# haileys/mixlab

Hardware: AMD Instinct MI355X
Metric: audio_ch_mixed_per_sec (higher is better)
Workload: dtype f32 (f64 intermediates); 1 GPU; 1024-channel Mixer + EqThree + Envelope chain (Trigger->Envelope; noise->EqThree->StereoPanner->Amplifier->Mixer), 48000 Hz f32; strips=1024, gates=toggle every 30 ticks, phase k mod 60, applied between ticks inside the batch, eq_mode=exact order: speculative time-parallel kernel, verified bit-exact, parallelism=strips sharded x1, ticks_policy=one GPU

## Files before the change

include/mixlab_gpu.h:

```cpp
#ifndef MIXLAB_GPU_H
#define MIXLAB_GPU_H

#include <stddef.h>
#include <stdint.h>

#ifdef __cplusplus
extern "C" {
#endif

#define MX_ABI_VERSION 4u

enum {
    MX_OK = 0,
    MX_ERR_INVALID = -1,
    MX_ERR_TYPE = -2,
    MX_ERR_DEVICE = -3,
    MX_ERR_NOMEM = -4,
    MX_ERR_INTERNAL = -5,
    MX_ERR_FULL = -6
};

typedef enum { MX_DISCONNECTED = 0, MX_MONO = 1, MX_STEREO = 2, MX_VIDEO = 3 } mx_line;

enum {
// ... 11 lines not shown
    MX_KIND_SOURCE_MONO = 11,
    MX_KIND_SOURCE_STEREO = 12,
    MX_KIND_SOURCE_VIDEO = 13,
    MX_KIND_VIDEO_TO_RGBA = 14,
    MX_KIND_FIR = 15,
    MX_KIND_RESAMPLE = 16,
    MX_KIND_MONITOR = 17,
    MX_KIND_OUTPUT_DEVICE = 18,
    MX_KIND_COUNT = 19
};
#define MX_PROFILE_KINDS 18

enum { MX_WAVE_ON = 0, MX_WAVE_OFF = 1, MX_WAVE_SINE = 2, MX_WAVE_SQUARE = 3, MX_WAVE_TRIANGLE = 4, MX_WAVE_SAW = 5 };

typedef struct { double gain_db; double fader; uint8_t cue; uint8_t _pad[7]; } mx_mixer_channel_params;
typedef struct { double gain_lo_db, gain_mid_db, gain_hi_db; } mx_eq_three_params;
typedef struct { double attack_ms, decay_ms, sustain_amplitude, release_ms; } mx_envelope_params;
typedef struct { double amplitude, mod_depth; } mx_amplifier_params;
typedef struct { double freq; uint32_t waveform; uint32_t _pad; } mx_oscillator_params;
typedef struct { double freq_lo, freq_hi; } mx_fm_sine_params;
typedef struct { uint32_t gate_open; } mx_trigger_params;
typedef struct { int32_t a, b;  double fader; } mx_video_mixer_params;
typedef struct { int32_t use_matrix; int32_t matrix_q12[12]; } mx_video_to_rgba_params;
typedef struct { uint32_t width, height; } mx_monitor_params;
typedef struct { uint32_t width, height, queue_depth, _pad; } mx_monitor_params_ex;
typedef struct { uint32_t channels; int32_t left, right; uint32_t _pad; } mx_output_device_params;
typedef struct { uint32_t n_taps; uint32_t _pad;  } mx_fir_params;
typedef struct { uint32_t up, down, taps_per_phase, _pad;  } mx_resample_params;

typedef struct { uint32_t kind; uint32_t params_len; const void* params; } mx_node;
typedef struct { uint32_t src_node, src_port, dst_node, dst_port; } mx_edge;

#define MX_FLAG_EQ_EXACT 1u
#define MX_FLAG_EQ_FAST 4u
#define MX_FLAG_FP_CONTRACT 16u

#define MX_FLAG_OVERLAP_TAIL 8u
#define MX_FLAG_NO_FUSE 2u

typedef struct {
    uint32_t sample_rate;
    uint32_t ticks_per_second;
    uint32_t max_ticks_per_run;
    uint32_t flags;
    int32_t device;
    int32_t _pad;
    void* stream;
} mx_graph_opts;

typedef struct mx_graph mx_graph;

const char* mx_last_error(void);
uint32_t mx_abi_version(void);
int mx_device_count(void);

int mx_graph_build(const mx_node* nodes, size_t n_nodes, const mx_edge* edges, size_t n_edges,
                   const mx_graph_opts* opts, mx_graph** out);
void mx_graph_destroy(mx_graph* g);

int mx_graph_samples_per_tick(const mx_graph* g, size_t* spt);
int mx_graph_run_order(const mx_graph* g, uint32_t* order, size_t cap, size_t* n);

int mx_graph_stream(mx_graph* g, void** stream);
int mx_graph_tail_stream(mx_graph* g, void** stream);

int mx_graph_update_params(mx_graph* g, uint32_t node, const void* params, size_t params_len);

typedef struct { uint32_t node; uint32_t tick_in_run; const void* params; size_t params_len; } mx_param_event;
int mx_graph_schedule_params(mx_graph* g, uint32_t node, uint32_t tick_in_run, const void* params, size_t params_len);
int mx_graph_schedule_params_batch(mx_graph* g, const mx_param_event* events, size_t n_events);

int mx_graph_eq_spec_stats(mx_graph* g, uint64_t* chunks_run, uint64_t* chunks_repaired);
int mx_graph_eq_repair_stats(mx_graph* g, uint64_t out[8]);
int mx_graph_debug_eq_records(mx_graph* g, void** device_records, size_t* bytes);
int mx_graph_debug_tail_releases(mx_graph* g, uint64_t* gated, uint64_t* at_once);
#define MX_EQ_LAUNCH_NONE 0u
#define MX_EQ_LAUNCH_SEQUENTIAL 1u
#define MX_EQ_LAUNCH_DIRECT 2u
#define MX_EQ_LAUNCH_TILED 3u
#define MX_EQ_LAUNCH_RAGGED_TICK 4u
#define MX_EQ_LAUNCH_CONTROL_TILE 5u
#define MX_EQ_LAUNCH_SCAN 6u
int mx_graph_debug_eq_launch(mx_graph* g, uint32_t out[5]);

int mx_graph_write_source(mx_graph* g, uint32_t node, const float* host_samples, size_t n_ticks);
int mx_graph_bind_source_device(mx_graph* g, uint32_t node, const void* device_ptr);

int mx_graph_run_ticks(mx_graph* g, uint64_t first_tick, uint32_t n_ticks);
int mx_graph_sync(mx_graph* g);

int mx_graph_read_output(mx_graph* g, uint32_t node, uint32_t port, float* host_samples, size_t n_ticks);
int mx_graph_read_output_window(mx_graph* g, uint32_t node, uint32_t port, float* host_samples, size_t first_tick_in_run, size_t n_ticks);
int mx_graph_read_output_i16(mx_graph* g, uint32_t node, uint32_t port, int16_t* host_samples, size_t n_ticks);
int mx_graph_write_source_i16(mx_graph* g, uint32_t node, const int16_t* host_samples, size_t n_ticks);

int mx_graph_output_device_ptr(mx_graph* g, uint32_t node, uint32_t port, void** device_ptr, size_t* floats_per_tick);

typedef struct { uint8_t clip, clip_status, lag_status, changed; uint32_t channels; } mx_audio_out_tick;
int mx_graph_read_audio_out(mx_graph* g, uint32_t node, uint32_t first_tick_in_run, uint32_t n_ticks, float* samples, size_t samples_cap,
                            mx_audio_out_tick* ticks, size_t* n_samples);
int mx_graph_audio_out_lag(mx_graph* g, uint32_t node);

typedef struct { uint32_t node, port; } mx_port_ref;
typedef struct { uint32_t hold_ticks; float release; } mx_meter_params;
typedef struct {
    float    peak[2];
    float    hold[2];
    double   sum_sq[2];
    uint32_t over[2];
    uint32_t frames;
    uint32_t channels;
} mx_meter_tick;
int mx_graph_set_meters(mx_graph* g, const mx_port_ref* ports, size_t n, const mx_meter_params* params);
int mx_graph_read_meters(mx_graph* g, uint32_t first_tick_in_run, uint32_t n_ticks, mx_meter_tick* dst, size_t cap);

typedef struct {
    uint32_t        n_fft;
    uint32_t        n_bands;
    const uint16_t* edges;
} mx_spectrum_params;
int mx_graph_set_spectra(mx_graph* g, const mx_port_ref* ports, size_t n, const mx_spectrum_params* params);
int mx_graph_read_spectra(mx_graph* g, uint32_t first_tick_in_run, uint32_t n_ticks, float* dst, size_t cap);
int mx_spectrum_tables(uint32_t n_fft, float* window, float* twiddle_re, float* twiddle_im);

typedef struct { uint32_t momentary_ticks; uint32_t short_ticks; } mx_loudness_params;
typedef struct {
    double   ksq[2];
    double   momentary_sq;
    double   short_sq;
    float    true_peak[2];
    uint32_t frames;
    uint32_t channels;
} mx_loudness_tick;
int mx_graph_set_loudness(mx_graph* g, const mx_port_ref* ports, size_t n, const mx_loudness_params* params);
int mx_graph_read_loudness(mx_graph* g, uint32_t first_tick_in_run, uint32_t n_ticks, mx_loudness_tick* dst, size_t cap);
int mx_loudness_tables(double rate, uint32_t frames_per_tick, double* biquads, double* carry, float* interp);
int mx_loudness_gate(const double* block_sq, const uint32_t* block_frames, size_t n_blocks, double* lufs_integrated, size_t* blocks_kept);

typedef struct { uint32_t window_ticks , grid , zoom_log2 , hop ; } mx_stereo_params;
typedef struct {
    double   sum_ll;
    double   sum_rr;
    double   sum_lr;
    double   win_ll;
    double   win_rr;
    double   win_lr;
    uint32_t frames;
    uint32_t nonfinite;
} mx_stereo_tick;
int mx_graph_set_stereo(mx_graph* g, const mx_port_ref* ports, size_t n, const mx_stereo_params* params);
int mx_graph_read_stereo(mx_graph* g, uint32_t first_tick_in_run, uint32_t n_ticks, mx_stereo_tick* dst, size_t cap);
int mx_graph_read_goniometers(mx_graph* g, void* dst, size_t cap_bytes, uint32_t* n_records);
int mx_stereo_gonio_record_bytes(const mx_stereo_params* params, size_t* bytes);
int mx_stereo_correlation(double ll, double rr, double lr, double* r);

typedef struct { float ceiling; uint32_t lookahead; } mx_limiter_params;
#define MX_LIMITER_MAX_LOOKAHEAD 512u
typedef struct {
    float    min_gain;
    float    peak_out;
    uint32_t limited;
    uint32_t nonfinite;
    uint32_t frames;
    uint32_t channels;
} mx_limiter_tick;
int mx_graph_set_limiters(mx_graph* g, const mx_port_ref* ports, size_t n, const mx_limiter_params* params);
// ... 227 lines not shown
```

mixlab_amd/abi.py:

```python
from __future__ import annotations

import ctypes as C
import pathlib

import numpy as np

_PKG = pathlib.Path(__file__).resolve().parent
LIB_PATH = _PKG / "libmixlab_gpu.so"

if not LIB_PATH.exists():
    raise ImportError(
        f"{LIB_PATH} is missing: build it with `python -m mixlab_amd.build` (hipcc, gfx950). "
        "mixlab_amd has no CPU fallback."
    )

lib = C.CDLL(str(LIB_PATH))

MX_OK, MX_ERR_INVALID, MX_ERR_TYPE, MX_ERR_DEVICE, MX_ERR_NOMEM, MX_ERR_INTERNAL, MX_ERR_FULL = 0, -1, -2, -3, -4, -5, -6
MX_DISCONNECTED, MX_MONO, MX_STEREO, MX_VIDEO = 0, 1, 2, 3
(KIND_AMPLIFIER, KIND_ENVELOPE, KIND_EQ_THREE, KIND_FM_SINE, KIND_MIXER, KIND_OSCILLATOR, KIND_PLOTTER,
 KIND_STEREO_PANNER, KIND_STEREO_SPLITTER, KIND_TRIGGER, KIND_VIDEO_MIXER, KIND_SOURCE_MONO,
 KIND_SOURCE_STEREO, KIND_SOURCE_VIDEO, KIND_VIDEO_TO_RGBA, KIND_FIR, KIND_RESAMPLE, KIND_MONITOR, KIND_OUTPUT_DEVICE, KIND_COUNT) = range(20)
PROFILE_KINDS = 18
KIND_NAMES = ["amplifier", "envelope", "eq_three", "fm_sine", "mixer", "oscillator", "plotter", "stereo_panner",
# ... 7 lines not shown
FLAG_OVERLAP_TAIL = 8
EQ_LAUNCH = {0: "none", 1: "sequential", 2: "direct", 3: "tiled", 4: "ragged_tick", 5: "control_tile", 6: "scan"}


class MixerChannelParams(C.Structure):
    _fields_ = [("gain_db", C.c_double), ("fader", C.c_double), ("cue", C.c_uint8), ("_pad", C.c_uint8 * 7)]


class EqThreeParams(C.Structure):
    _fields_ = [("gain_lo_db", C.c_double), ("gain_mid_db", C.c_double), ("gain_hi_db", C.c_double)]


class EnvelopeParams(C.Structure):
    _fields_ = [("attack_ms", C.c_double), ("decay_ms", C.c_double), ("sustain_amplitude", C.c_double), ("release_ms", C.c_double)]


class AmplifierParams(C.Structure):
    _fields_ = [("amplitude", C.c_double), ("mod_depth", C.c_double)]


class OscillatorParams(C.Structure):
    _fields_ = [("freq", C.c_double), ("waveform", C.c_uint32), ("_pad", C.c_uint32)]


class FmSineParams(C.Structure):
    _fields_ = [("freq_lo", C.c_double), ("freq_hi", C.c_double)]


class TriggerParams(C.Structure):
    _fields_ = [("gate_open", C.c_uint32)]


class Node(C.Structure):
    _fields_ = [("kind", C.c_uint32), ("params_len", C.c_uint32), ("params", C.c_void_p)]


class Edge(C.Structure):
    _fields_ = [("src_node", C.c_uint32), ("src_port", C.c_uint32), ("dst_node", C.c_uint32), ("dst_port", C.c_uint32)]


class GraphOpts(C.Structure):
    _fields_ = [("sample_rate", C.c_uint32), ("ticks_per_second", C.c_uint32), ("max_ticks_per_run", C.c_uint32),
                ("flags", C.c_uint32), ("device", C.c_int32), ("_pad", C.c_int32), ("stream", C.c_void_p)]


class Frame(C.Structure):
    _fields_ = [("width", C.c_uint32), ("height", C.c_uint32), ("data", C.c_void_p * 3), ("stride", C.c_int32 * 3),
                ("dur_num", C.c_int64), ("dur_den", C.c_int64), ("off_num", C.c_int64), ("off_den", C.c_int64)]


class Input(C.Structure):
    _fields_ = [("kind", C.c_int), ("samples", C.c_void_p), ("len", C.c_size_t), ("video", C.c_void_p)]


class Output(C.Structure):
    _fields_ = [("kind", C.c_int), ("samples", C.c_void_p), ("len", C.c_size_t), ("video", C.c_void_p), ("video_present", C.c_int)]


def _proto(name, restype, *argtypes):
    fn = getattr(lib, name)
    fn.restype = restype
    fn.argtypes = list(argtypes)
    return fn


_proto("mx_last_error", C.c_char_p)
_proto("mx_abi_version", C.c_uint32)
_proto("mx_device_count", C.c_int)
_proto("mx_graph_build", C.c_int, C.POINTER(Node), C.c_size_t, C.POINTER(Edge), C.c_size_t, C.POINTER(GraphOpts), C.POINTER(C.c_void_p))
_proto("mx_graph_destroy", None, C.c_void_p)
_proto("mx_graph_samples_per_tick", C.c_int, C.c_void_p, C.POINTER(C.c_size_t))
_proto("mx_graph_run_order", C.c_int, C.c_void_p, C.POINTER(C.c_uint32), C.c_size_t, C.POINTER(C.c_size_t))
_proto("mx_graph_update_params", C.c_int, C.c_void_p, C.c_uint32, C.c_void_p, C.c_size_t)
class ParamEvent(C.Structure):
    _fields_ = [("node", C.c_uint32), ("tick_in_run", C.c_uint32), ("params", C.c_void_p), ("params_len", C.c_size_t)]


_proto("mx_graph_schedule_params", C.c_int, C.c_void_p, C.c_uint32, C.c_uint32, C.c_void_p, C.c_size_t)
_proto("mx_graph_schedule_params_batch", C.c_int, C.c_void_p, C.POINTER(ParamEvent), C.c_size_t)
_proto("mx_graph_eq_spec_stats", C.c_int, C.c_void_p, C.POINTER(C.c_uint64), C.POINTER(C.c_uint64))
_proto("mx_graph_debug_eq_records", C.c_int, C.c_void_p, C.POINTER(C.c_void_p), C.POINTER(C.c_size_t))
_proto("mx_graph_debug_tail_releases", C.c_int, C.c_void_p, C.POINTER(C.c_uint64), C.POINTER(C.c_uint64))
_proto("mx_graph_debug_eq_launch", C.c_int, C.c_void_p, C.POINTER(C.c_uint32))
_proto("mx_graph_eq_repair_stats", C.c_int, C.c_void_p, C.POINTER(C.c_uint64))
_proto("mx_graph_write_source", C.c_int, C.c_void_p, C.c_uint32, C.c_void_p, C.c_size_t)
_proto("mx_graph_bind_source_device", C.c_int, C.c_void_p, C.c_uint32, C.c_void_p)
_proto("mx_graph_run_ticks", C.c_int, C.c_void_p, C.c_uint64, C.c_uint32)
_proto("mx_graph_sync", C.c_int, C.c_void_p)
_proto("mx_graph_read_output", C.c_int, C.c_void_p, C.c_uint32, C.c_uint32, C.c_void_p, C.c_size_t)
_proto("mx_graph_read_output_window", C.c_int, C.c_void_p, C.c_uint32, C.c_uint32, C.c_void_p, C.c_size_t, C.c_size_t)
_proto("mx_graph_read_output_i16", C.c_int, C.c_void_p, C.c_uint32, C.c_uint32, C.c_void_p, C.c_size_t)
_proto("mx_graph_write_source_i16", C.c_int, C.c_void_p, C.c_uint32, C.c_void_p, C.c_size_t)
_proto("mx_graph_output_device_ptr", C.c_int, C.c_void_p, C.c_uint32, C.c_uint32, C.POINTER(C.c_void_p), C.POINTER(C.c_size_t))
_proto("mx_graph_tail_stream", C.c_int, C.c_void_p, C.POINTER(C.c_void_p))
_proto("mx_graph_stream", C.c_int, C.c_void_p, C.POINTER(C.c_void_p))
_proto("mx_graph_read_plotter", C.c_int, C.c_void_p, C.c_uint32, C.c_uint32, C.c_void_p, C.c_void_p, C.POINTER(C.c_int))
class OutputDeviceParams(C.Structure):
    _fields_ = [("channels", C.c_uint32), ("left", C.c_int32), ("right", C.c_int32), ("_pad", C.c_uint32)]


class AudioOutTick(C.Structure):
    _fields_ = [("clip", C.c_uint8), ("clip_status", C.c_uint8), ("lag_status", C.c_uint8), ("changed", C.c_uint8), ("channels", C.c_uint32)]


AUDIO_OUT_TICK_DTYPE = np.dtype([("clip", np.uint8), ("clip_status", np.uint8), ("lag_status", np.uint8), ("changed", np.uint8), ("channels", np.uint32)])
_proto("mx_graph_read_audio_out", C.c_int, C.c_void_p, C.c_uint32, C.c_uint32, C.c_uint32, C.c_void_p, C.c_size_t, C.c_void_p, C.POINTER(C.c_size_t))
_proto("mx_graph_audio_out_lag", C.c_int, C.c_void_p, C.c_uint32)
class PortRef(C.Structure):
    _fields_ = [("node", C.c_uint32), ("port", C.c_uint32)]


class MeterParams(C.Structure):
    _fields_ = [("hold_ticks", C.c_uint32), ("release", C.c_float)]


METER_TICK_DTYPE = np.dtype({"names": ["peak", "hold", "sum_sq", "over", "frames", "channels"],
                             "formats": [(np.float32, 2), (np.float32, 2), (np.float64, 2), (np.uint32, 2), np.uint32, np.uint32],
                             "offsets": [0, 8, 16, 32, 40, 44], "itemsize": 48})
_proto("mx_graph_set_meters", C.c_int, C.c_void_p, C.c_void_p, C.c_size_t, C.c_void_p)
_proto("mx_graph_read_meters", C.c_int, C.c_void_p, C.c_uint32, C.c_uint32, C.c_void_p, C.c_size_t)
class SpectrumParams(C.Structure):
    _fields_ = [("n_fft", C.c_uint32), ("n_bands", C.c_uint32), ("edges", C.POINTER(C.c_uint16))]


_proto("mx_graph_set_spectra", C.c_int, C.c_void_p, C.c_void_p, C.c_size_t, C.c_void_p)
_proto("mx_graph_read_spectra", C.c_int, C.c_void_p, C.c_uint32, C.c_uint32, C.c_void_p, C.c_size_t)
_proto("mx_spectrum_tables", C.c_int, C.c_uint32, C.c_void_p, C.c_void_p, C.c_void_p)
class LoudnessParams(C.Structure):
    _fields_ = [("momentary_ticks", C.c_uint32), ("short_ticks", C.c_uint32)]


LOUDNESS_TICK_DTYPE = np.dtype({"names": ["ksq", "momentary_sq", "short_sq", "true_peak", "frames", "channels"],
                                "formats": [(np.float64, 2), np.float64, np.float64, (np.float32, 2), np.uint32, np.uint32],
                                "offsets": [0, 16, 24, 32, 40, 44], "itemsize": 48})
_proto("mx_graph_set_loudness", C.c_int, C.c_void_p, C.c_void_p, C.c_size_t, C.c_void_p)
_proto("mx_graph_read_loudness", C.c_int, C.c_void_p, C.c_uint32, C.c_uint32, C.c_void_p, C.c_size_t)
_proto("mx_loudness_tables", C.c_int, C.c_double, C.c_uint32, C.c_void_p, C.c_void_p, C.c_void_p)
_proto("mx_loudness_gate", C.c_int, C.c_void_p, C.c_void_p, C.c_size_t, C.POINTER(C.c_double), C.POINTER(C.c_size_t))
class StereoParams(C.Structure):
    _fields_ = [("window_ticks", C.c_uint32), ("grid", C.c_uint32), ("zoom_log2", C.c_uint32), ("hop", C.c_uint32)]


STEREO_TICK_DTYPE = np.dtype({"names": ["sum_ll", "sum_rr", "sum_lr", "win_ll", "win_rr", "win_lr", "frames", "nonfinite"],
                              "formats": [np.float64] * 6 + [np.uint32] * 2,
                              "offsets": [0, 8, 16, 24, 32, 40, 48, 52], "itemsize": 56})
_proto("mx_graph_set_stereo", C.c_int, C.c_void_p, C.c_void_p, C.c_size_t, C.c_void_p)
_proto("mx_graph_read_stereo", C.c_int, C.c_void_p, C.c_uint32, C.c_uint32, C.c_void_p, C.c_size_t)
_proto("mx_graph_read_goniometers", C.c_int, C.c_void_p, C.c_void_p, C.c_size_t, C.POINTER(C.c_uint32))
_proto("mx_stereo_gonio_record_bytes", C.c_int, C.POINTER(StereoParams), C.POINTER(C.c_size_t))
_proto("mx_stereo_correlation", C.c_int, C.c_double, C.c_double, C.c_double, C.POINTER(C.c_double))
class LimiterParams(C.Structure):
    _fields_ = [("ceiling", C.c_float), ("lookahead", C.c_uint32)]


LIMITER_MAX_LOOKAHEAD = 512
LIMITER_TILE = 2048
LIMITER_TICK_DTYPE = np.dtype({"names": ["min_gain", "peak_out", "limited", "nonfinite", "frames", "channels"],
                               "formats": [np.float32, np.float32, np.uint32, np.uint32, np.uint32, np.uint32],
                               "offsets": [0, 4, 8, 12, 16, 20], "itemsize": 24})
_proto("mx_graph_set_limiters", C.c_int, C.c_void_p, C.c_void_p, C.c_size_t, C.c_void_p)
_proto("mx_graph_read_limiters", C.c_int, C.c_void_p, C.c_uint32, C.c_uint32, C.c_void_p, C.c_size_t)
_proto("mx_graph_read_limited", C.c_int, C.c_void_p, C.c_size_t, C.c_uint32, C.c_uint32, C.c_void_p, C.c_size_t, C.POINTER(C.c_size_t))
_proto("mx_graph_read_limited_i16", C.c_int, C.c_void_p, C.c_size_t, C.c_uint32, C.c_uint32, C.c_void_p, C.c_size_t, C.POINTER(C.c_size_t))
_proto("mx_graph_limited_device_ptr", C.c_int, C.c_void_p, C.c_size_t, C.POINTER(C.c_void_p), C.POINTER(C.c_size_t))
_proto("mx_limiter_weights", C.c_int, C.c_uint32, C.c_void_p)
class TempoParams(C.Structure):
# ... 242 lines not shown

def check(rc: int) -> None:
    if rc != MX_OK:
        raise MxError(rc, (lib.mx_last_error() or b"").decode("utf-8", "replace"))


def params_bytes(p) -> bytes:
    if p is None:
        return b""
    if isinstance(p, (bytes, bytearray)):
        return bytes(p)
    if isinstance(p, (list, tuple)):
        return b"".join(bytes(x) for x in p)
    return bytes(p)


class Graph:

    def __init__(self, nodes, edges, sample_rate=44100, ticks_per_second=60, max_ticks_per_run=1, flags=0,
                 device=-1, stream=None):
        self._h = C.c_void_p()
        blobs = [params_bytes(p) for (_k, p) in nodes]
        self._keep = []
        n_arr = (Node * max(1, len(nodes)))()
        for i, ((kind, _p), blob) in enumerate(zip(nodes, blobs)):
            buf = C.create_string_buffer(blob, len(blob)) if blob else None
            self._keep.append(buf)
            n_arr[i] = Node(kind, len(blob), C.cast(buf, C.c_void_p) if buf else None)
        e_arr = (Edge * max(1, len(edges)))()
        for i, e in enumerate(edges):
            e_arr[i] = Edge(*e)
        opts = GraphOpts(sample_rate, ticks_per_second, max_ticks_per_run, flags, device, 0, stream)
        check(lib.mx_graph_build(n_arr, len(nodes), e_arr, len(edges), C.byref(opts), C.byref(self._h)))
        spt = C.c_size_t()
        check(lib.mx_graph_samples_per_tick(self._h, C.byref(spt)))
        self.spt = spt.value
        self.max_ticks = max_ticks_per_run
        self.n_nodes = len(nodes)

    def close(self):
        if getattr(self, "_h", None) is not None and self._h.value:
            lib.mx_graph_destroy(self._h)
            self._h = C.c_void_p()

    def __del__(self):
        try:
            self.close()
        except Exception:
            pass

    def run_order(self):
        n = C.c_size_t()
        arr = (C.c_uint32 * max(1, self.n_nodes))()
        check(lib.mx_graph_run_order(self._h, arr, self.n_nodes, C.byref(n)))
        return list(arr[: n.value])

    def update_params(self, node, params):
        blob = params_bytes(params)
        check(lib.mx_graph_update_params(self._h, node, blob, len(blob)))

    def schedule_params(self, node, tick_in_run: int, params):
        blob = params_bytes(params)
        check(lib.mx_graph_schedule_params(self._h, node, tick_in_run, blob, len(blob)))

    def schedule_params_batch(self, events: "C.Array", n: int | None = None):
        check(lib.mx_graph_schedule_params_batch(self._h, events, len(events) if n is None else n))

    def eq_repair_stats(self) -> dict:
        v = (C.c_uint64 * 8)()
        check(lib.mx_graph_eq_repair_stats(self._h, v))
        keys = ("chunks_run", "chunks_repaired", "settled_by_comparison", "walk_steps_16", "fill_steps_16", "island_rounds", "in_order_walks", "nan_fills")
        return {k: int(x) for k, x in zip(keys, v)}

    def debug_tail_releases(self):
        a, b = C.c_uint64(), C.c_uint64()
        check(lib.mx_graph_debug_tail_releases(self._h, C.byref(a), C.byref(b)))
        return a.value, b.value

    def debug_eq_launch(self) -> dict:
        v = (C.c_uint32 * 5)()
        check(lib.mx_graph_debug_eq_launch(self._h, v))
        return {"form": EQ_LAUNCH.get(v[0], str(v[0])), "super_block": int(v[1]), "n_chunks": int(v[2]), "chunk": int(v[3]), "warm": int(v[4])}

    def debug_eq_records(self):
        p, n = C.c_void_p(), C.c_size_t()
        check(lib.mx_graph_debug_eq_records(self._h, C.byref(p), C.byref(n)))
        return p.value, n.value

    def eq_spec_stats(self):
        a, b = C.c_uint64(), C.c_uint64()
        check(lib.mx_graph_eq_spec_stats(self._h, C.byref(a), C.byref(b)))
        return a.value, b.value

    def write_source(self, node, samples: np.ndarray, n_ticks: int):
        a = np.ascontiguousarray(samples, dtype=np.float32)
        check(lib.mx_graph_write_source(self._h, node, a.ctypes.data_as(C.c_void_p), n_ticks))

    def bind_source_device(self, node, device_ptr: int):
        check(lib.mx_graph_bind_source_device(self._h, node, C.c_void_p(device_ptr)))

    def run_ticks(self, first_tick: int, n_ticks: int = 1):
        check(lib.mx_graph_run_ticks(self._h, first_tick, n_ticks))

    def sync(self):
        check(lib.mx_graph_sync(self._h))

    def read_output(self, node, port, n_ticks: int, stereo: bool, rate=(1, 1)) -> np.ndarray:
        out = np.empty(n_ticks * (self.spt * rate[0] // rate[1]) * (2 if stereo else 1), dtype=np.float32)
        check(lib.mx_graph_read_output(self._h, node, port, out.ctypes.data_as(C.c_void_p), n_ticks))
        return out

    def read_output_window(self, node, port, first_tick: int, n_ticks: int, stereo: bool) -> np.ndarray:
        out = np.empty(n_ticks * self.spt * (2 if stereo else 1), dtype=np.float32)
        check(lib.mx_graph_read_output_window(self._h, node, port, out.ctypes.data_as(C.c_void_p), first_tick, n_ticks))
        return out

    def read_audio_out(self, node, first_tick: int, n_ticks: int):
        n = C.c_size_t(0)
        check(lib.mx_graph_read_audio_out(self._h, node, first_tick, n_ticks, None, 0, None, C.byref(n)))
        samples = np.empty(n.value, dtype=np.float32)
        ticks = np.empty(n_ticks, dtype=AUDIO_OUT_TICK_DTYPE)
        check(lib.mx_graph_read_audio_out(self._h, node, first_tick, n_ticks, samples.ctypes.data_as(C.c_void_p), n.value,
                                          ticks.ctypes.data_as(C.c_void_p), C.byref(n)))
        return samples, ticks

    def audio_out_lag(self, node):
        check(lib.mx_graph_audio_out_lag(self._h, node))

    def set_meters(self, ports, params=MeterParams(0, 1.0)):
        ports = list(ports)
        if isinstance(params, MeterParams):
            params = [params] * len(ports)
        pa = (PortRef * max(1, len(ports)))(*[PortRef(int(n), int(p)) for (n, p) in ports])
        pr = (MeterParams * max(1, len(ports)))(*[MeterParams(q.hold_ticks, q.release) for q in params])
        check(lib.mx_graph_set_meters(self._h, pa, len(ports), pr))
        self._n_meters = len(ports)

    def read_meters(self, first_tick: int, n_ticks: int) -> np.ndarray:
        n = getattr(self, "_n_meters", 0)
        out = np.zeros((n_ticks, n), dtype=METER_TICK_DTYPE)
        check(lib.mx_graph_read_meters(self._h, first_tick, n_ticks, out.ctypes.data_as(C.c_void_p), out.size))
        return out

    def set_spectra(self, ports, n_fft: int = 2048, edges=None):
        ports = list(ports)
        if not ports:
            check(lib.mx_graph_set_spectra(self._h, None, 0, None))
            self._spectra = (0, 0)
            return
        e = np.ascontiguousarray(edges, dtype=np.uint16)
        if e.ndim != 1 or e.size < 2 or not np.array_equal(e, np.asarray(edges)):
            raise ValueError("edges: at least two bin indices that fit 16 bits")
        pa = (PortRef * len(ports))(*[PortRef(int(n), int(p)) for (n, p) in ports])
        pr = SpectrumParams(int(n_fft), e.size - 1, e.ctypes.data_as(C.POINTER(C.c_uint16)))
        check(lib.mx_graph_set_spectra(self._h, pa, len(ports), C.byref(pr)))
        self._spectra = (len(ports), e.size - 1)

    def read_spectra(self, first_tick: int, n_ticks: int) -> np.ndarray:
        n, b = getattr(self, "_spectra", (0, 0))
        out = np.zeros((n_ticks, n, 2, b), dtype=np.float32)
        check(lib.mx_graph_read_spectra(self._h, first_tick, n_ticks, out.ctypes.data_as(C.c_void_p), out.size))
        return out

    def set_loudness(self, ports, momentary_ticks: int = 24, short_ticks: int = 180):
        ports = list(ports)
        if not ports:
# ... 258 lines not shown
```

mixlab_amd/csrc/mx_abi.cpp:

```cpp
#include <cmath>
#include <cstring>
#include <memory>
#include <string>

#include "mx_engine.hpp"

using mx::Error;
using mx::Graph;

struct mx_graph { std::unique_ptr<Graph> g; };

struct mx_module {
    uint32_t kind = 0;
    std::unique_ptr<Graph> g;
    std::unique_ptr<mx::VideoMixer> vm;
    uint32_t tps = 60;
    std::vector<uint8_t> in_type, out_type;
};

static thread_local std::string t_last_error;
void mx_set_last_error(const std::string& s) { t_last_error = s; }

template <class F>
static int guard(F&& f) noexcept {
// ... 26 lines not shown
    int n = 0;
    hipError_t e = hipGetDeviceCount(&n);
    if (e != hipSuccess) { t_last_error = std::string("hipGetDeviceCount: ") + hipGetErrorString(e); (void)hipGetLastError(); return MX_ERR_DEVICE; }
    return n;
}

int mx_graph_build(const mx_node* nodes, size_t n_nodes, const mx_edge* edges, size_t n_edges,
                   const mx_graph_opts* opts, mx_graph** out) {
    return guard([&] {
        REQUIRE(out, "out is NULL");
        *out = nullptr;
        mx_graph_opts o{};
        o.device = -1;
        if (opts) o = *opts;
        auto h = std::make_unique<mx_graph>();
        h->g = std::make_unique<Graph>(nodes, n_nodes, edges, n_edges, o);
        *out = h.release();
    });
}

void mx_graph_destroy(mx_graph* g) {
    (void)guard([&] { delete g; });
}

int mx_graph_samples_per_tick(const mx_graph* g, size_t* spt) {
    return guard([&] { REQUIRE(g && spt, "NULL argument"); *spt = g->g->spt(); });
}

int mx_graph_run_order(const mx_graph* g, uint32_t* order, size_t cap, size_t* n) {
    return guard([&] {
        REQUIRE(g && n, "NULL argument");
        const auto& o = g->g->run_order();
        *n = o.size();
        for (size_t i = 0; i < o.size() && i < cap && order; ++i) order[i] = o[i];
    });
}

int mx_graph_stream(mx_graph* g, void** stream) {
    return guard([&] { REQUIRE(g && stream, "NULL argument"); *stream = (void*)g->g->stream(); });
}
int mx_graph_tail_stream(mx_graph* g, void** stream) {
    return guard([&] { REQUIRE(g && stream, "NULL argument"); *stream = (void*)g->g->tail_stream(); });
}
int mx_graph_update_params(mx_graph* g, uint32_t node, const void* params, size_t params_len) {
    return guard([&] { REQUIRE(g, "graph is NULL"); g->g->update_params(node, params, params_len); });
}

int mx_graph_schedule_params(mx_graph* g, uint32_t node, uint32_t tick_in_run, const void* params, size_t params_len) {
    return guard([&] { REQUIRE(g, "graph is NULL"); g->g->schedule_params(node, tick_in_run, params, params_len); });
}

int mx_graph_schedule_params_batch(mx_graph* g, const mx_param_event* events, size_t n_events) {
    return guard([&] {
        REQUIRE(g, "graph is NULL");
        REQUIRE(events || !n_events, "events is NULL");
        for (size_t i = 0; i < n_events; ++i) g->g->check_schedule(events[i].node, events[i].params, events[i].params_len);
        for (size_t i = 0; i < n_events; ++i) g->g->schedule_params(events[i].node, events[i].tick_in_run, events[i].params, events[i].params_len);
    });
}

int mx_graph_eq_spec_stats(mx_graph* g, uint64_t* chunks_run, uint64_t* chunks_repaired) {
    return guard([&] {
        REQUIRE(g, "graph is NULL");
        uint64_t v[8];
        g->g->eq_spec_stats(v);
        if (chunks_run) *chunks_run = v[0];
        if (chunks_repaired) *chunks_repaired = v[1];
    });
}

int mx_graph_debug_eq_records(mx_graph* g, void** device_records, size_t* bytes) {
    return guard([&] {
        REQUIRE(g && device_records, "NULL argument");
        g->g->sync();
        *device_records = g->g->debug_eq_records(bytes);
    });
}
int mx_graph_debug_tail_releases(mx_graph* g, uint64_t* gated, uint64_t* at_once) {
    return guard([&] { REQUIRE(g, "NULL argument"); g->g->tail_releases(gated, at_once); });
}

int mx_graph_debug_eq_launch(mx_graph* g, uint32_t out[5]) {
    return guard([&] { REQUIRE(g && out, "NULL argument"); g->g->eq_launch(out); });
}

int mx_graph_eq_repair_stats(mx_graph* g, uint64_t out[8]) {
    return guard([&] {
        REQUIRE(g, "graph is NULL");
        REQUIRE(out, "out is NULL");
        g->g->eq_spec_stats(out);
    });
}

int mx_graph_write_source(mx_graph* g, uint32_t node, const float* host_samples, size_t n_ticks) {
    return guard([&] { REQUIRE(g, "graph is NULL"); g->g->write_source(node, host_samples, n_ticks * g->g->spt()); });
}

int mx_graph_bind_source_device(mx_graph* g, uint32_t node, const void* device_ptr) {
    return guard([&] { REQUIRE(g, "graph is NULL"); g->g->bind_source(node, device_ptr); });
}

int mx_graph_run_ticks(mx_graph* g, uint64_t first_tick, uint32_t n_ticks) {
    return guard([&] {
        REQUIRE(g, "graph is NULL");
        try {
            g->g->run(first_tick * (uint64_t)g->g->spt(), g->g->spt(), n_ticks);
        } catch (...) {
            g->g->drop_schedules();
            throw;
        }
    });
}

int mx_graph_sync(mx_graph* g) {
    return guard([&] { REQUIRE(g, "graph is NULL"); g->g->sync(); });
}

int mx_graph_read_output(mx_graph* g, uint32_t node, uint32_t port, float* host_samples, size_t n_ticks) {
    return guard([&] { REQUIRE(g, "graph is NULL"); g->g->read_output(node, port, host_samples, n_ticks * g->g->spt()); });
}

int mx_graph_read_output_window(mx_graph* g, uint32_t node, uint32_t port, float* host_samples, size_t first_tick_in_run, size_t n_ticks) {
    return guard([&] {
        REQUIRE(g, "graph is NULL");
        g->g->read_output(node, port, host_samples, n_ticks * g->g->spt(), first_tick_in_run * g->g->spt());
    });
}

int mx_graph_read_output_i16(mx_graph* g, uint32_t node, uint32_t port, int16_t* host_samples, size_t n_ticks) {
    return guard([&] { REQUIRE(g, "graph is NULL"); g->g->read_output_i16(node, port, host_samples, n_ticks * g->g->spt()); });
}

int mx_graph_write_source_i16(mx_graph* g, uint32_t node, const int16_t* host_samples, size_t n_ticks) {
    return guard([&] { REQUIRE(g, "graph is NULL"); g->g->write_source_i16(node, host_samples, n_ticks * g->g->spt()); });
}

int mx_graph_output_device_ptr(mx_graph* g, uint32_t node, uint32_t port, void** device_ptr, size_t* floats_per_tick) {
    return guard([&] {
        REQUIRE(g && device_ptr, "NULL argument");
        size_t fpf = 0;
        *device_ptr = g->g->output_ptr(node, port, &fpf);
        if (floats_per_tick) *floats_per_tick = fpf;
    });
}

int mx_graph_read_audio_out(mx_graph* g, uint32_t node, uint32_t first_tick_in_run, uint32_t n_ticks, float* samples, size_t samples_cap,
                            mx_audio_out_tick* ticks, size_t* n_samples) {
    static_assert(sizeof(mx_audio_out_tick) == sizeof(mx::OutTick), "mx_audio_out_tick is the device record");
    return guard([&] {
        REQUIRE(g, "graph is NULL");
        g->g->read_audio_out(node, first_tick_in_run, n_ticks, samples, samples_cap, reinterpret_cast<mx::OutTick*>(ticks), n_samples);
    });
}

int mx_graph_audio_out_lag(mx_graph* g, uint32_t node) {
    return guard([&] { REQUIRE(g, "graph is NULL"); g->g->audio_out_lag(node); });
}

int mx_graph_set_meters(mx_graph* g, const mx_port_ref* ports, size_t n, const mx_meter_params* params) {
    return guard([&] { REQUIRE(g, "graph is NULL"); g->g->meters().set(ports, n, params); });
}

int mx_graph_read_meters(mx_graph* g, uint32_t first_tick_in_run, uint32_t n_ticks, mx_meter_tick* dst, size_t cap) {
    static_assert(sizeof(mx_meter_tick) == 48 && sizeof(mx_meter_tick) == sizeof(mx::MeterTick), "mx_meter_tick is the device record");
    static_assert(offsetof(mx_meter_tick, sum_sq) == offsetof(mx::MeterTick, sum_sq) && offsetof(mx_meter_tick, frames) == offsetof(mx::MeterTick, frames),
                  "mx_meter_tick is the device record");
// ... 500 lines not shown
```

mixlab_amd/csrc/mx_engine.cpp:

```cpp
#include <chrono>

#include "mx_engine.hpp"

#include <cstdio>

#include <algorithm>
#include <cmath>
#include <cstring>

namespace mx {

void hip_check(hipError_t e, const char* what) {
    if (e != hipSuccess) throw Error(MX_ERR_DEVICE, std::string(what) + ": " + hipGetErrorString(e));
}

void DevBuf::alloc(size_t n) {
    free_();
    if (n == 0) n = 256;
    hipError_t e = hipMalloc(&p, n);
    if (e == hipErrorOutOfMemory) { p = nullptr; throw Error(MX_ERR_NOMEM, "hipMalloc: out of device memory"); }
    hip_check(e, "hipMalloc");
    bytes = n;
}
void DevBuf::free_() {
// ... 194 lines not shown
    for (Node& n : nodes_) n.sub_key = eq_key(n);
    std::vector<uint32_t> sorted;
    for (uint32_t id : order_) if (!nodes_[id].elided && nodes_[id].kind != MX_KIND_OUTPUT_DEVICE) sorted.push_back(id);
    for (uint32_t id : order_) if (nodes_[id].kind == MX_KIND_OUTPUT_DEVICE) od_nodes_.push_back(id);
    std::stable_sort(sorted.begin(), sorted.end(), [&](uint32_t a, uint32_t b) {
        if (nodes_[a].level != nodes_[b].level) return nodes_[a].level < nodes_[b].level;
        if (nodes_[a].kind != nodes_[b].kind) return nodes_[a].kind < nodes_[b].kind;
        if (nodes_[a].sub_key != nodes_[b].sub_key) return nodes_[a].sub_key < nodes_[b].sub_key;
        const uint64_t da = ((uint64_t)nodes_[a].dom_num << 32) | nodes_[a].dom_den, db = ((uint64_t)nodes_[b].dom_num << 32) | nodes_[b].dom_den;
        return da < db;
    });
    for (uint32_t id : sorted) {
        Node& n = nodes_[id];
        if (groups_.empty() || groups_.back().level != n.level || groups_.back().kind != n.kind || groups_.back().sub_key != n.sub_key ||
            groups_.back().dom_num != n.dom_num || groups_.back().dom_den != n.dom_den ||
            groups_.back().in_dom_num != n.in_dom_num || groups_.back().in_dom_den != n.in_dom_den) {
            Group g; g.level = n.level; g.kind = n.kind; g.sub_key = n.sub_key;
            g.dom_num = n.dom_num; g.dom_den = n.dom_den; g.in_dom_num = n.in_dom_num; g.in_dom_den = n.in_dom_den;
            groups_.push_back(std::move(g));
        }
        n.group = (int)groups_.size() - 1;
        n.slot = (uint32_t)groups_.back().nodes.size();
        groups_.back().nodes.push_back(id);
    }
    for (uint32_t id = 0; id < nodes_.size(); ++id) if (nodes_[id].kind == MX_KIND_PLOTTER && nodes_[id].group >= 0) plotter_nodes_.push_back(id);
    for (uint32_t id : order_) if (nodes_[id].kind == MX_KIND_VIDEO_MIXER || nodes_[id].kind == MX_KIND_SOURCE_VIDEO || nodes_[id].kind == MX_KIND_VIDEO_TO_RGBA || nodes_[id].kind == MX_KIND_MONITOR) video_order_.push_back(id);
    for (Node& n : nodes_) {
        if (n.kind == MX_KIND_VIDEO_MIXER) {
            mx_video_mixer_params p; std::memcpy(&p, n.params.data(), sizeof p);
            n.vmixer.reset(new VideoMixer(p, sr, stream_));
        }
        if (n.kind == MX_KIND_MONITOR) {
            mx_monitor_params p; std::memcpy(&p, n.params.data(), sizeof p);
            if (p.width == 0 || p.height == 0 || (p.width & 1) || (p.height & 1) || p.width > 16384 || p.height > 16384)
                throw Error(MX_ERR_INVALID, "monitor picture must be non-zero, even and at most 16384 a side");
            n.mon_scaler = std::make_shared<Scaler>(p.width, p.height, stream_);
            if (n.params.size() == sizeof(mx_monitor_params_ex)) { mx_monitor_params_ex px; std::memcpy(&px, n.params.data(), sizeof px); n.mon_depth = px.queue_depth; }
            const uint64_t kept = (uint64_t)(n.mon_depth ? n.mon_depth : std::max<uint32_t>(1u, o.max_ticks_per_run)) * (((uint64_t)p.width + 63) & ~63ull) * p.height * 3 / 2;
            if (kept > (64ull << 30)) throw Error(MX_ERR_NOMEM, "a Monitor that keeps every tick of a submission would hold more than 64 GiB of pictures: give it a queue depth (mx_monitor_params_ex) or fewer ticks per run");
        }
        if (n.kind == MX_KIND_VIDEO_MIXER || n.kind == MX_KIND_SOURCE_VIDEO || n.kind == MX_KIND_VIDEO_TO_RGBA || n.kind == MX_KIND_MONITOR) has_video_ = true;
        n.vout.resize(n.out_type.size());
    }
    if (!(flags_ & MX_FLAG_NO_FUSE)) {
        std::vector<uint32_t> n_cons(nodes_.size(), 0); std::vector<uint8_t> ok(nodes_.size(), 1);
        for (const Node& n : nodes_)
            for (const PortRef& pr : n.in_src)
                if (pr.node >= 0 && nodes_[pr.node].kind == MX_KIND_VIDEO_MIXER && pr.port == 0) {
                    n_cons[pr.node]++;
                    if (n.kind != MX_KIND_VIDEO_MIXER && n.kind != MX_KIND_VIDEO_TO_RGBA) ok[pr.node] = 0;
                }
        for (size_t i = 0; i < nodes_.size(); ++i)
            if (nodes_[i].vmixer) { nodes_[i].vlazy = n_cons[i] == 1 && ok[i]; nodes_[i].vmixer->set_lazy_program(nodes_[i].vlazy, tps); }
    }
    {
        std::vector<EqScanTab> tabs(4);
        const long double fs[2] = {(long double)lo_f_, (long double)hi_f_};
        for (int v = 0; v < 4; ++v) {
            const uint64_t L = 4ull << v;
            for (int f = 0; f < 2; ++f) {
                for (int j = 0; j <= 64; ++j) toeplitz_pow(fs[f], L * (uint64_t)j, tabs[v].pw[f][j]);
                for (int k = 0; k < 6; ++k) toeplitz_pow(fs[f], L << k, tabs[v].p2[f][k]);
                const long double ff = fs[f], vsa = 1.0L / 4294967295.0L;
                const long double b[4] = {ff, ff * ff, ff * ff * ff, ff * ff * ff * ff};
                const long double c[4] = {vsa, vsa * ff, vsa * ff * ff, vsa * ff * ff * ff};
                long double sum[4] = {0, 0, 0, 0};
                for (uint64_t m = 0; m < 32; ++m) {
                    long double am[4], hb[4];
                    toeplitz_pow_ld(ff, m, am);
                    toeplitz_apply_ld(am, b, hb);
                    for (int q = 0; q < 4; ++q) tabs[v].h[f][m][q] = (double)hb[q];
                    if (m < L) for (int q = 0; q < 4; ++q) sum[q] += am[q];
                }
                long double cz[4];
                toeplitz_apply_ld(sum, c, cz);
                for (int q = 0; q < 4; ++q) tabs[v].cz[f][q] = (double)cz[q];
            }
        }
        eq_tabs_.alloc(tabs.size() * sizeof(EqScanTab));
        hip_check(hipMemcpy(eq_tabs_.p, tabs.data(), tabs.size() * sizeof(EqScanTab), hipMemcpyHostToDevice), "hipMemcpy(eq tabs)");
    }
    { const char* const sm = getenv("MX_SIN_MODE"); sin_mode_ = sm ? atoi(sm) : 0; }
    { const char* const gt = getenv("MX_TAIL_GATE_TEST"); gate_test_ = gt && atoi(gt); }
    bool overlap_auto = false;
    {
        const char* const ae = getenv("MX_OVERLAP_AUTO");
        const bool auto_on = !(ae && atoi(ae) == 0);
        const size_t max_ticks = spt_ ? cap_frames_ / spt_ : 0;
        size_t n_eq = 0;
        for (const Group& g : groups_) if (g.kind == MX_KIND_EQ_THREE) n_eq = std::max(n_eq, g.nodes.size());
        overlap_auto = auto_on && eq_exact() && n_eq >= 64 && max_ticks >= 16;
    }
    size_t t_first = groups_.size();
    while (t_first > 0 && groups_[t_first - 1].kind == MX_KIND_MIXER) --t_first;
    if (((flags_ & MX_FLAG_OVERLAP_TAIL) || overlap_auto) && !has_video_ && groups_.size() >= 2 && t_first >= 1 && t_first < groups_.size() &&
        groups_[t_first - 1].level < groups_[t_first].level && plotter_nodes_.empty()) {
        bool ok = true;
        std::vector<std::pair<uint32_t, uint32_t>> ports;
        for (size_t tg = t_first; tg < groups_.size() && ok; ++tg)
            for (uint32_t id : groups_[tg].nodes) {
                for (const PortRef& pr : nodes_[id].in_src) {
                    if (pr.node < 0) continue;
                    const Node& sn = nodes_[pr.node];
                    if (sn.group >= (int)t_first && sn.group < (int)tg) continue;
                    if (sn.kind == MX_KIND_SOURCE_MONO || sn.kind == MX_KIND_SOURCE_STEREO || sn.group >= (int)tg) { ok = false; break; }
                    if (std::find(ports.begin(), ports.end(), std::make_pair((uint32_t)pr.node, (uint32_t)pr.port)) == ports.end()) ports.push_back({(uint32_t)pr.node, pr.port});
                }
                if (!ok) break;
            }
        if (ok && overlap_auto && !(flags_ & MX_FLAG_OVERLAP_TAIL)) {
            const char* const ge = getenv("MX_OVERLAP_AUTO_MAX_GB");
            const double max_gb = ge ? atof(ge) : 32.0;
            size_t free_b = 0, total_b = 0;
            if (hipMemGetInfo(&free_b, &total_b) != hipSuccess) free_b = 0;
            const double extra = (double)ports.size() * (double)cap_frames_ * 8.0;
            if (extra > max_gb * 1073741824.0 || extra > (double)free_b / 4.0) ok = false;
        }
        if (ok) {
            tail_gi_ = (int)t_first;
            tail_auto_ = !(flags_ & MX_FLAG_OVERLAP_TAIL);
            for (auto& pp : ports) nodes_[pp.first].out_off2[pp.second] = 0;
            hip_check(hipStreamCreateWithFlags(&tail_stream_, hipStreamNonBlocking), "hipStreamCreate(tail)");
            hip_check(hipEventCreateWithFlags(&ev_head_done_, hipEventDisableTiming), "hipEventCreate");
            for (auto& e : ev_tail_done_) hip_check(hipEventCreateWithFlags(&e, hipEventDisableTiming), "hipEventCreate");
        }
    }
    layout_slab();
    build_descriptors();
    for (Node& n : nodes_) {
        if (n.kind != MX_KIND_OUTPUT_DEVICE) continue;
        n.od_frames = (uint32_t)(spt_ * n.in_dom_num / n.in_dom_den);
        const OutState st0{-1, -1, 0u, 0u};
        n.od_state.alloc(sizeof(OutState));
        hip_check(hipMemcpy(n.od_state.p, &st0, sizeof st0, hipMemcpyHostToDevice), "hipMemcpy(output device state)");
        n.od_rec.alloc(std::max<size_t>(1, cap_frames_ / spt_) * sizeof(OutTick));
        od_update(n);
        hip_check(hipStreamSynchronize(stream_), "hipStreamSynchronize");
    }
}

void Graph::od_grow(Node& n, uint32_t channels) {
    if (channels <= n.od_cmax) return;
    const size_t F = n.od_frames, ticks = std::max<size_t>(1, cap_frames_ / spt_);
    DevBuf sc; sc.alloc(F * channels * sizeof(float));
    hip_check(hipMemsetAsync(sc.p, 0, F * channels * sizeof(float), stream_), "hipMemsetAsync(output device scratch)");
    if (n.od_cmax) hip_check(hipMemcpyAsync(sc.p, n.od_scratch.p, F * n.od_cmax * sizeof(float), hipMemcpyDeviceToDevice, stream_), "hipMemcpyAsync(output device scratch)");
    hip_check(hipStreamSynchronize(stream_), "hipStreamSynchronize");
    n.od_scratch = std::move(sc);
    n.od_out.alloc(ticks * F * channels * sizeof(float));
    n.od_part.alloc(ticks * out_route_blocks(F, channels) * sizeof(uint32_t));
    n.od_cmax = channels;
}

void Graph::od_update(Node& n) {
    mx_output_device_params p; std::memcpy(&p, n.params.data(), sizeof p);
    n.od_channels = p.channels;
    if (!p.channels) return;
    od_grow(n, p.channels);
    if (n.od_left != p.left || n.od_right != p.right)
        hip_check(hipMemsetAsync(n.od_scratch.p, 0, (size_t)n.od_frames * n.od_cmax * sizeof(float), stream_), "hipMemsetAsync(output device scratch)");
    n.od_left = p.left >= 0 && (uint32_t)p.left < p.channels ? p.left : -1;
    n.od_right = p.right >= 0 && (uint32_t)p.right < p.channels ? p.right : -1;
}

size_t Graph::od_offset(const Node& n, uint32_t tick) const {
    size_t off = 0;
// ... 699 lines not shown
    } else {
        cuts.push_back(n_calls);
        uint32_t from = 0;
        for (uint32_t to : cuts) {
            if (from) {
                apply_at(from);
                sync();
                run_off_frames_ = (size_t)from * fpc;
                build_descriptors();
            }
            run_span(t0 + (uint64_t)from * fpc, fpc, from, to - from, n_calls);
            from = to;
        }
        sync();
        run_off_frames_ = 0;
        build_descriptors();
    }
    if (any_sched) {
        for (uint32_t sid : sched_nodes_) {
            Node& n = nodes_[sid];
            if (!n.gate_sched.empty()) {
                mx_trigger_params tp{}; tp.gate_open = n.gate_sched.back().second;
                std::memcpy(n.params.data(), &tp, sizeof tp);
                ++gates_version_;
                n.gate_sched.clear();
            }
            n.sched.clear();
        }
        sched_nodes_.clear();
    }
    hip_check(hipGetLastError(), "kernel launch");
    last_calls_ = n_calls;
    last_frames_per_call_ = fpc;
    for (AudioTapSet* s : taps_) s->run_ticks = s->empty() ? 0u : n_calls;
    if (prof) ++prof_runs_count_;
    if (ms_by_kind) (void)profile_collect(ms_by_kind, ms_total);
}

void Graph::run_span(uint64_t t0, size_t fpc, uint32_t call_off, uint32_t n_calls, uint32_t run_calls) {
    const size_t frames = fpc * (size_t)n_calls;
    ProfSpan* prof = nullptr;
    if (prof_this_run_) {
        if (prof_pool_.empty()) prof_pool_.push_back(std::make_unique<ProfSpan>(groups_.size()));
        prof = prof_pool_.back().get();
        prof->tail_held = prof->od = prof->od_tail = prof->meters = prof->meters_tail = false;
        hip_check(hipEventRecord(prof->begin, stream_), "hipEventRecord");
    }
    std::vector<PlotJob> jobs;
    size_t gi = 0;
    bool first_eq = true;
    for (Group& g : groups_) {
        const uint32_t n = (uint32_t)g.nodes.size();
        const size_t gf = frames * g.dom_num / g.dom_den;
        const size_t gfpc = fpc * g.dom_num / g.dom_den;
        const GateBits gates{(const uint32_t*)g.gates.p, g.gate_words, call_off};
        switch (g.kind) {
        case MX_KIND_AMPLIFIER: launch_amplifier((const AmpDesc*)desc_of(g), n, gf, stream_, fp_contract()); break;
        case MX_KIND_ENVELOPE: {
            const size_t need = envelope_scratch_bytes(n, gf);
            if (need && (g.spec.bytes < need || !g.spec.p)) { sync(); g.spec.alloc(need); }
            launch_envelope((const EnvDesc*)desc_of(g), (EnvState*)g.state.p, n, gf, gfpc, gates, t0, sample_rate_, stream_, fp_contract(), need ? g.spec.p : nullptr, need ? g.spec.bytes : 0);
            break;
        }
        case MX_KIND_EQ_THREE: {
            EqRun r{gf, gfpc, n_calls, fp_contract() ? 1u : 0u, t0, sample_rate_, 1.0 / sample_rate_, lo_f_, hi_f_, nullptr};
            uint32_t launch[5] = {MX_EQ_LAUNCH_SEQUENTIAL, 0u, 1u, (uint32_t)gf, 0u};
            if (g.state2.p) {
                const size_t need = (size_t)n * n_calls * sizeof(EnvTick);
                if (g.env_ticks.bytes < need || !g.env_ticks.p) { sync(); g.env_ticks.alloc(need); }
                launch_env_ticks((const EnvTickDesc*)g.tick_desc.p, n, gates, n_calls, gfpc, t0, sample_rate_, (EnvTick*)g.env_ticks.p, stream_, fp_contract());
                r.ticks = (const EnvTick*)g.env_ticks.p;
            }
            if (eq_exact()) {
                EqSpecPlan plan;
                if (eq_plan_spec(n, gf, gfpc, lo_f_, hi_f_, plan, g.eq_mode == 6 || g.eq_mode == 7, g.eq_mode == 4 || g.eq_mode == 5)) {
                    const size_t need = eq_spec_scratch_bytes(n, plan);
                    if (g.spec.bytes < need || !g.spec.p) { sync(); g.spec.alloc(need); }
                    if (!eq_stats_.p) { eq_stats_.alloc(8 * sizeof(uint64_t)); hip_check(hipMemset(eq_stats_.p, 0, 8 * sizeof(uint64_t)), "hipMemset"); }
                    gate_armed_ = false;
                    if (deferred_.pending) {
                        if (!gate_flag_.p) { gate_flag_.alloc(64); hip_check(hipMemset(gate_flag_.p, 0, 64), "hipMemset"); }
                        r.started = (uint32_t*)gate_flag_.p; r.started_seq = ++gate_seq_; gate_armed_ = true;
                    }
                    const bool opens_gate = launch_eq_three_spec((const EqDesc*)desc_of(g), (EqState*)g.state.p, n, r, plan, g.eq_mode, g.spec.p, (uint64_t*)eq_stats_.p, stream_, launch);
                    if (!opens_gate && !gate_test_) gate_armed_ = false;
                    if (deferred_.pending) flush_deferred_tail(true);
                } else {
                    void* scratch = nullptr;
                    if (eq_use_poles_split(n, gf)) {
                        const size_t need = eq_poles_scratch_bytes(n, gf);
                        if (g.spec.bytes < need || !g.spec.p) { sync(); g.spec.alloc(need); }
                        scratch = g.spec.p;
                    }
                    launch_eq_three_exact((const EqDesc*)desc_of(g), (EqState*)g.state.p, n, r, scratch, stream_);
                    launch[1] = scratch ? 2u : 1u;
                }
            } else {
                EqSplit sp{1u, 5u, 0u, 0u, gf, gf, nullptr, nullptr, nullptr};
                EqSpanPow pp{};
                eq_plan_split(n, gf, lo_f_, hi_f_, sp);
                if (sp.n_split > 1) {
                    const size_t need = (size_t)n * sp.n_split * 8 * sizeof(double) + (size_t)n * 12 * sizeof(double);
                    if (g.extra.bytes < need || !g.extra.p) { sync(); g.extra.alloc(need); }
                    sp.zbuf = (double*)g.extra.p;
                    sp.bound = sp.zbuf + (size_t)n * sp.n_split * 8;
                    toeplitz_pow((long double)lo_f_, sp.span, pp.lo);
                    toeplitz_pow((long double)hi_f_, sp.span, pp.hi);
                }
                launch_eq_three_scan((const EqDesc*)desc_of(g), (EqState*)g.state.p, n, r, (const EqScanTab*)eq_tabs_.p, sp, pp, stream_);
                launch[0] = MX_EQ_LAUNCH_SCAN; launch[2] = sp.n_split; launch[3] = (uint32_t)sp.span; launch[4] = (uint32_t)sp.warm;
            }
            if (first_eq) { std::copy(launch, launch + 5, eq_launch_); first_eq = false; }
            break;
        }
        case MX_KIND_FM_SINE: launch_fm_sine((const FmDesc*)desc_of(g), n, gf, t0, sample_rate_, stream_, sin_mode_); break;
        case MX_KIND_MIXER:
            if (overlap_this_run_ && (int)gi >= tail_gi_) {
                if ((int)gi == tail_gi_) {
                    if (deferred_.pending) flush_deferred_tail(false);
                    hip_check(hipEventRecord(ev_head_done_, stream_), "hipEventRecord");
                    deferred_.items.clear(); deferred_.outs.clear(); deferred_.taps.clear(); deferred_.parity = parity_; deferred_.prof = prof;
                    if (prof) prof->tail_held = true;
                }
                deferred_.items.push_back(TailLaunch{desc_of(g), n, g.max_taps, gf, g.dup_mode, prof ? prof->group_end[gi] : nullptr});
                if (gi + 1 == groups_.size()) deferred_.pending = true;
                ++gi;
                continue;
            }
            launch_mixer((const MixDesc*)desc_of(g), n, g.max_taps , gf, g.dup_mode, stream_);
            break;
        case MX_KIND_OSCILLATOR: launch_oscillator((const OscDesc*)desc_of(g), n, gf, t0, sample_rate_, stream_, sin_mode_); break;
        case MX_KIND_STEREO_PANNER: launch_panner((const PanDesc*)desc_of(g), n, gf, stream_); break;
        case MX_KIND_STEREO_SPLITTER: launch_splitter((const SplitDesc*)desc_of(g), n, gf, stream_); break;
        case MX_KIND_TRIGGER: launch_trigger((const TrigDesc*)desc_of(g), n, gf, gfpc, &gates, stream_); break;
        case MX_KIND_FIR: launch_fir((const FirDesc*)desc_of(g), n, g.max_taps, gf, stream_, fp_contract()); break;
        case MX_KIND_RESAMPLE:
            launch_resample((const ResampleDesc*)desc_of(g), n, g.max_taps, g.rs_tab_doubles, g.rs_win_frames, frames * g.in_dom_num / g.in_dom_den, gf,
                            t0 * g.in_dom_num / g.in_dom_den, t0 * g.dom_num / g.dom_den, stream_, g.rs_common_up, fp_contract(), g.rs_common_taps, g.rs_common_down);
            break;
        case MX_KIND_PLOTTER: {
            jobs.clear();
            for (uint32_t id : g.nodes) {
                const Node& nd = nodes_[id];
                for (uint32_t c = 0; c < n_calls; ++c) {
                    if (!nd.plot_fired[call_off + c]) continue;
                    float* stage = (float*)plot_stage_.p + (size_t)nd.plot_slot[call_off + c] * 2 * fpc;
                    jobs.push_back(PlotJob{in_ptr(nd, 0, false, parity_) + (size_t)c * 2 * fpc, stage, stage + fpc});
                }
            }
            if (!jobs.empty()) {
                PlotJob* dst = (PlotJob*)plot_jobs_.p + plot_job_off_;
                stage_upload(dst, jobs.data(), jobs.size() * sizeof(PlotJob));
                launch_plotter(dst, (uint32_t)jobs.size(), fpc, stream_);
                plot_job_off_ += jobs.size();
            }
            break;
        }
        default: break;
        }
        if (prof && group_launches(g)) hip_check(hipEventRecord(prof->group_end[gi], stream_), "hipEventRecord");
        ++gi;
    }
    if (has_video_) {
        for (uint32_t c = 0; c < n_calls; ++c) { video_tick_in_run_ = call_off + c; run_video_tick(t0 + (uint64_t)c * fpc); }
        flush_scales(stream_);
        for (uint32_t id : video_order_) { Node& vn = nodes_[id]; if (!vn.rgba_pending.empty()) launch_pending_rgba(vn, vn.rgba_pending.size(), false); vn.rgba_calls = 0; }
    }
    if (prof && has_video_) hip_check(hipEventRecord(prof->video_end, stream_), "hipEventRecord");
    launch_outputs(t0, call_off, n_calls, prof);
    if (call_off + n_calls == run_calls) for (AudioTapSet* s : taps_) launch_tap_set(*s, run_calls, prof);
    if (prof) { prof_runs_.push_back(std::move(prof_pool_.back())); prof_pool_.pop_back(); }
}

static bool group_launches(const Group& g) {
    switch (g.kind) {
    case MX_KIND_SOURCE_MONO: case MX_KIND_SOURCE_STEREO: case MX_KIND_SOURCE_VIDEO:
    case MX_KIND_VIDEO_MIXER: case MX_KIND_VIDEO_TO_RGBA: case MX_KIND_MONITOR: return false;
    default: return true;
    }
}

void Graph::profile_enable(bool on) { prof_on_ = on; }

Graph::ProfSpan::ProfSpan(size_t n_groups) : group_end(n_groups) {
    for (hipEvent_t* e : {&begin, &video_end, &tail_begin, &od_end, &od_tail_end, &meters_end, &meters_tail_end}) hip_check(hipEventCreate(e), "hipEventCreate");
    for (hipEvent_t& e : group_end) hip_check(hipEventCreate(&e), "hipEventCreate");
}

Graph::ProfSpan::~ProfSpan() {
    for (hipEvent_t e : {begin, video_end, tail_begin, od_end, od_tail_end, meters_end, meters_tail_end}) (void)hipEventDestroy(e);
    for (hipEvent_t e : group_end) (void)hipEventDestroy(e);
}

uint32_t Graph::profile_collect(float* ms_by_kind, float* ms_total) {
    sync();
// ... 255 lines not shown
        if (C != 0 && C != 64 && C != 128 && C != 256) throw Error(MX_ERR_INVALID, "mx_video_scope_params: wave_cols must be 0, 64, 128 or 256");
        if (params->hop == 0) throw Error(MX_ERR_INVALID, "mx_video_scope_params: hop must be >= 1");
    }
    std::vector<uint64_t> keys(n);
    for (size_t i = 0; i < n; ++i) {
        const mx_port_ref pr = ports[i];
        if (pr.node >= nodes_.size() || pr.port >= nodes_[pr.node].out_type.size()) throw Error(MX_ERR_INVALID, "video scope: output terminal out of range");
        if (nodes_[pr.node].out_type[pr.port] != MX_VIDEO) throw Error(MX_ERR_TYPE, "video scope: an audio port has no picture (meters and spectrum taps observe audio ports)");
        keys[i] = (uint64_t)pr.node << 32 | pr.port;
    }
    std::sort(keys.begin(), keys.end());
    if (std::adjacent_find(keys.begin(), keys.end()) != keys.end()) throw Error(MX_ERR_INVALID, "video scope: duplicate (node, port)");
    size_t rec_bytes = 0, cap = 0;
    if (n) {
        rec_bytes = scope_record_bytes(params->wave_cols, params->vectorscope);
        const size_t max_ticks = std::max<size_t>(1, cap_frames_ / spt_);
        cap = (max_ticks + params->hop - 1) / params->hop;
        const unsigned __int128 need = (unsigned __int128)cap * n * rec_bytes;
        if (need > ((unsigned __int128)4 << 30))
            throw Error(MX_ERR_NOMEM, "video scopes: the records of one run (ceil(max_ticks_per_run / hop) x taps x record bytes) exceed 4 GiB: raise hop");
    }
    sync();
    scopes_.assign(ports, ports + n);
    scope_c_ = 0; scope_n_ = 0; scope_run_seen_ = false; scope_now_ = false;
    scope_rec_.free_();
    scope_rec_bytes_ = rec_bytes; scope_cap_ = cap;
    if (scopes_.empty()) { scope_par_ = mx_video_scope_params{0, 0, 1}; return; }
    scope_par_ = *params;
    scope_rec_.alloc(cap * n * rec_bytes);
}

size_t Graph::read_video_scopes(void* dst, size_t cap_bytes) {
    hip_check(hipSetDevice(device_), "hipSetDevice");
    if (scopes_.empty()) throw Error(MX_ERR_INVALID, "no video scope taps are set");
    if (!scope_run_seen_) throw Error(MX_ERR_INVALID, "no run since the video scope taps were set");
    const size_t count = (size_t)scope_n_ * scopes_.size(), bytes = count * scope_rec_bytes_;
    if (cap_bytes < bytes) throw Error(MX_ERR_INVALID, "cap_bytes is smaller than recorded ticks x taps x record bytes");
    if (bytes && !dst) throw Error(MX_ERR_INVALID, "dst is NULL");
    if (bytes) {
        wait_tail(-1);
        hip_check(hipMemcpyAsync(dst, scope_rec_.p, bytes, hipMemcpyDeviceToHost, stream_), "hipMemcpyAsync(D2H)");
        sync();
    }
    return count;
}

void Graph::read_output_i16(uint32_t node, uint32_t port, int16_t* host, size_t frames) {
    hip_check(hipSetDevice(device_), "hipSetDevice");
    wait_tail(-1);
    if (node >= nodes_.size() || port >= nodes_[node].out_type.size()) throw Error(MX_ERR_INVALID, "output terminal out of range");
    if (frames > cap_frames_) throw Error(MX_ERR_INVALID, "more ticks than max_ticks_per_run");
    if (frames && !host) throw Error(MX_ERR_INVALID, "host_samples is NULL");
    const Node& n = nodes_[node];
    if (n.out_elided[port]) throw Error(MX_ERR_INVALID, "port is not materialised: it only feeds a fused consumer (build with MX_FLAG_NO_FUSE to observe it)");
    const size_t cnt = floats_per_frame(n.out_type[port]) * (frames * n.dom_num / n.dom_den);
    if (!cnt) return;
    if (conv_stage_.bytes < cnt * sizeof(int16_t)) { sync(); conv_stage_.alloc(cnt * sizeof(int16_t)); }
    launch_f32_to_i16(out_ptr(n, port, parity_), (int16_t*)conv_stage_.p, cnt, n.out_dup[port] ? 1 : 0, stream_);
    hip_check(hipMemcpyAsync(host, conv_stage_.p, cnt * sizeof(int16_t), hipMemcpyDeviceToHost, stream_), "hipMemcpyAsync(D2H i16)");
    sync();
}

void Graph::write_source_i16(uint32_t node, const int16_t* host, size_t frames) {
    hip_check(hipSetDevice(device_), "hipSetDevice");
    if (node >= nodes_.size()) throw Error(MX_ERR_INVALID, "node out of range");
    Node& n = nodes_[node];
    if (n.kind != MX_KIND_SOURCE_MONO && n.kind != MX_KIND_SOURCE_STEREO) throw Error(MX_ERR_INVALID, "node is not a SOURCE_*");
    if (n.bound) throw Error(MX_ERR_INVALID, "source is bound to a caller device buffer");
    if (frames > cap_frames_) throw Error(MX_ERR_INVALID, "more ticks than max_ticks_per_run");
    if (frames && !host) throw Error(MX_ERR_INVALID, "host_samples is NULL");
    const size_t cnt = floats_per_frame(n.out_type[0]) * frames;
    if (!cnt) return;
    if (conv_stage_.bytes < cnt * sizeof(int16_t)) { sync(); conv_stage_.alloc(cnt * sizeof(int16_t)); }
    hip_check(hipMemcpyAsync(conv_stage_.p, host, cnt * sizeof(int16_t), hipMemcpyHostToDevice, stream_), "hipMemcpyAsync(H2D i16)");
    launch_i16_to_f32((const int16_t*)conv_stage_.p, out_ptr(n, 0, parity_), cnt, stream_);
    sync();
}

void* Graph::debug_eq_records(size_t* bytes) const {
    for (const Group& g : groups_)
        if (g.kind == MX_KIND_EQ_THREE && g.spec.p) { if (bytes) *bytes = g.spec.bytes; return g.spec.p; }
    if (bytes) *bytes = 0;
    return nullptr;
}

float* Graph::output_ptr(uint32_t node, uint32_t port, size_t* fpf, bool stream_ordered_consumer) {
    if (node >= nodes_.size() || port >= nodes_[node].out_type.size()) throw Error(MX_ERR_INVALID, "output terminal out of range");
    if (nodes_[node].out_elided[port]) throw Error(MX_ERR_INVALID, "port is not materialised: it only feeds a fused consumer (build with MX_FLAG_NO_FUSE to observe it)");
    if (nodes_[node].out_dup[port]) throw Error(MX_ERR_INVALID, "port is stored as one float per frame (L == R fused result): use mx_graph_read_output, or build with MX_FLAG_NO_FUSE");
    if (fpf) *fpf = floats_per_frame(nodes_[node].out_type[port]) * (spt_ * nodes_[node].dom_num / nodes_[node].dom_den);
    if (stream_ordered_consumer && tail_gi_ >= 0 && tail_auto_ && (nodes_[node].group >= tail_gi_ || nodes_[node].out_off2[port] != SIZE_MAX)) end_auto_tail();
    return out_ptr(nodes_[node], port, parity_);
}

int Graph::read_plotter(uint32_t node, uint32_t call, float* left, float* right) {
    if (node >= nodes_.size() || nodes_[node].kind != MX_KIND_PLOTTER) throw Error(MX_ERR_INVALID, "node is not a Plotter");
    const Node& n = nodes_[node];
    if (call >= n.plot_fired.size()) throw Error(MX_ERR_INVALID, "tick_in_run is outside the last run");
    if (!n.plot_fired[call]) return 0;
    const size_t fpc = last_frames_per_call_;
    const float* stage = (const float*)plot_stage_.p + (size_t)n.plot_slot[call] * 2 * fpc;
    hip_check(hipMemcpyAsync(left, stage, fpc * sizeof(float), hipMemcpyDeviceToHost, stream_), "hipMemcpyAsync(D2H)");
    hip_check(hipMemcpyAsync(right, stage + fpc, fpc * sizeof(float), hipMemcpyDeviceToHost, stream_), "hipMemcpyAsync(D2H)");
    sync();
    return 1;
}

void Graph::run_video_tick(uint64_t t) {
    scope_now_ = false;
    if (!scopes_.empty()) { scope_now_ = scope_c_ % scope_par_.hop == 0; ++scope_c_; }
    for (uint32_t id : video_order_) {
        Node& n = nodes_[id];
        switch (n.kind) {
        case MX_KIND_SOURCE_VIDEO: {
            n.vout[0] = Node::VOut{};
            const uint64_t tick = t / spt_;
            while (!n.vsrc_sched.empty() && n.vsrc_sched.front().tick < tick) n.vsrc_sched.pop_front();
            if (!n.vsrc_sched.empty()) {
                if (n.vsrc_sched.front().tick == tick) {
                    Node::VSched& e = n.vsrc_sched.front();
                    n.vout[0].frame = e.frame; n.vout[0].dur = e.dur; n.vout[0].off = e.off;
                    n.vsrc_sched.pop_front();
                }
            } else if (!n.vsrc_ring.empty()) {
                n.vout[0].frame = n.vsrc_ring[n.vsrc_ring_pos]; n.vout[0].dur = n.vsrc_dur; n.vout[0].off = n.vsrc_off;
                n.vsrc_ring_pos = (n.vsrc_ring_pos + 1) % n.vsrc_ring.size();
            } else if (n.vsrc && (n.vsrc_repeat || n.vsrc_pending)) {
                n.vout[0].frame = n.vsrc; n.vout[0].dur = n.vsrc_dur; n.vout[0].off = n.vsrc_off;
                n.vsrc_pending = false;
            }
            if (n.vband && n.vout[0].frame) {
                FrameRef o;
                for (auto& f : n.vband_pool) if (f->rc.load(std::memory_order_acquire) == 1) { o = f; break; }
                if (!o) {
                    if (n.vband_pool.size() >= 8) n.vband_pool.erase(n.vband_pool.begin());
                    n.vband_pool.push_back(FrameRef(DFrame::create(n.vband->full_w(), n.vband->band_rows(), stream_), false));
                    o = n.vband_pool.back();
                }
                n.vband->run(n.vout[0].frame.f, o.f, stream_);
                n.vout[0].frame = o;
            }
            if (n.vplace_on && n.vout[0].frame) n.vout[0].frame = placed_source_frame(id, n.vout[0].frame);
            else if (n.vkey_on && n.vout[0].frame) n.vout[0].frame = keyed_source_frame(id, n.vout[0].frame);
            break;
        }
        case MX_KIND_VIDEO_MIXER: {
            VideoInput in[4];
            for (int i = 0; i < 4; ++i) {
                const PortRef pr = n.in_src[i];
                if (pr.node < 0) continue;
                const Node::VOut& v = nodes_[pr.node].vout[pr.port];
                if (!v.frame) continue;
                in[i].frame = v.frame.f; in[i].duration_hint = v.dur; in[i].tick_offset = v.off;
            }
            FrameRef o, a, b;
            n.vmixer->run_tick(t, in, o, a, b);
            n.vout[0] = Node::VOut{o, Rational::make(1, (int64_t)tps_), Rational::make(0, 1)};
            mx_video_mixer_params p; std::memcpy(&p, n.params.data(), sizeof p);
            n.vout[1] = Node::VOut{}; n.vout[2] = Node::VOut{};
            if (a && p.a >= 0 && p.a < 4) n.vout[1] = Node::VOut{a, in[p.a].duration_hint, in[p.a].tick_offset};
            if (b && p.b >= 0 && p.b < 4) n.vout[2] = Node::VOut{b, in[p.b].duration_hint, in[p.b].tick_offset};
            break;
        }
        case MX_KIND_MONITOR: {
            Node::MonTick mt;
            const Rational absolute = Rational::make((int64_t)t, (int64_t)sample_rate_);
// ... 332 lines not shown
```

mixlab_amd/csrc/mx_engine.hpp:

```cpp
#pragma once
#include <algorithm>
#include <array>
#include <atomic>
#include <functional>
#include <hip/hip_runtime.h>

#include <cstdint>
#include <memory>
#include <string>
#include <deque>
#include <vector>

#include "mx_common.hpp"
#include "mx_kernels.hpp"
#include "mx_taps.hpp"
#include "mx_video.hpp"

namespace mx {

struct PortRef { int32_t node = -1; uint32_t port = 0; };

struct Node {
    uint32_t kind = 0;
    std::vector<uint8_t> params;
// ... 47 lines not shown
    bool mon_has_epoch = false; Rational mon_epoch;
    std::shared_ptr<Scaler> mon_scaler;
    DevBuf mon_pack;
    uint32_t od_channels = 0, od_cmax = 0; int32_t od_left = -1, od_right = -1; uint32_t od_frames = 0;
    DevBuf od_scratch;
    DevBuf od_state;
    DevBuf od_out, od_rec, od_part;
    std::unique_ptr<std::atomic<bool>> od_lag;
    bool od_lag_run = false;
    struct OdSpan { uint32_t first, n, channels; };
    std::vector<OdSpan> od_spans;
};

struct Group {
    int level = 0;
    uint32_t kind = 0;
    int sub_key = 0;
    uint32_t dom_num = 1, dom_den = 1, in_dom_num = 1, in_dom_den = 1;
    uint32_t max_taps = 0;
    uint32_t rs_common_taps = 0, rs_common_down = 0;
    uint32_t rs_common_up = 0;
    uint32_t rs_tab_doubles = 0, rs_win_frames = 0;
    std::vector<uint32_t> nodes;
    DevBuf desc;
    DevBuf desc_alt, extra_alt;
    DevBuf state;
    DevBuf extra;
    DevBuf state2;
    int dup_mode = 0;
    bool has_gates = false;
    DevBuf gates; uint32_t gate_words = 0; uint64_t gates_version = ~0ull; uint32_t gates_calls = 0;
    DevBuf tick_desc;
    DevBuf env_ticks;
    DevBuf spec;
    int eq_mode = -1;
};

class Graph final : public TapHost {
public:
    Graph(const mx_node* nodes, size_t n_nodes, const mx_edge* edges, size_t n_edges, const mx_graph_opts& opts,
          size_t cap_frames_override = 0);
    ~Graph();

    size_t spt() const { return spt_; }
    double sample_rate() const override { return sample_rate_; }
    size_t cap_frames() const override { return cap_frames_; }
    const std::vector<uint32_t>& run_order() const { return order_; }
    hipStream_t stream() const override { return stream_; }
    int device() const override { return device_; }
    uint32_t ticks_per_second() const { return tps_; }
    hipStream_t tail_stream() { if (tail_gi_ >= 0) flush_deferred_tail(false); return tail_gi_ >= 0 ? tail_stream_ : nullptr; }
    void* debug_eq_records(size_t* bytes) const;
    void join_tail() override { if (tail_gi_ >= 0) wait_tail(-1); }
    size_t n_nodes() const { return nodes_.size(); }
    bool eq_exact() const { return (flags_ & MX_FLAG_EQ_EXACT) || !(flags_ & MX_FLAG_EQ_FAST); }
    bool fp_contract() const { return (flags_ & MX_FLAG_FP_CONTRACT) != 0; }
    const Node& node(uint32_t i) const { return nodes_.at(i); }

    void update_params(uint32_t node, const void* params, size_t len);
    void schedule_params(uint32_t node, uint32_t tick_in_run, const void* params, size_t len);
    void check_schedule(uint32_t node, const void* params, size_t len) const;
    void drop_schedules();
    void eq_spec_stats(uint64_t out[8]);
    void write_source(uint32_t node, const float* host, size_t frames);
    void bind_source(uint32_t node, const void* dev);
    void run(uint64_t t0, size_t frames_per_call, uint32_t n_calls, float* ms_by_kind = nullptr, float* ms_total = nullptr);
    void sync() override;
    void profile_enable(bool on);
    uint32_t profile_collect(float* ms_by_kind, float* ms_total);
    void read_output(uint32_t node, uint32_t port, float* host, size_t frames, size_t first_frame = 0);
    void read_audio_out(uint32_t node, uint32_t first, uint32_t n, float* samples, size_t samples_cap, OutTick* ticks, size_t* n_samples);
    void audio_out_lag(uint32_t node);
    MeterTaps& meters() { return meters_; } SpectrumTaps& spectra() { return spectra_; } LoudnessTaps& loudness() { return loudness_; }
    StereoTaps& stereo() { return stereos_; } LimiterTaps& limiters() { return limiters_; } TempoTaps& tempo() { return tempos_; } TonalityTaps& tonality() { return tonalities_; }
    bool tap_port(mx_port_ref r, TapPort& t) const override; size_t tap_fpc() const override { return tap_fpc_; }
    void set_video_scopes(const mx_port_ref* ports, size_t n, const mx_video_scope_params* params);
    size_t read_video_scopes(void* dst, size_t cap_bytes);
    void read_output_i16(uint32_t node, uint32_t port, int16_t* host, size_t frames);
    void write_source_i16(uint32_t node, const int16_t* host, size_t frames);
    float* output_ptr(uint32_t node, uint32_t port, size_t* floats_per_tick, bool stream_ordered_consumer = true );
    bool tail_held() const { return deferred_.pending; }
    void tail_releases(uint64_t* gated, uint64_t* at_once) const { if (gated) *gated = n_gated_; if (at_once) *at_once = n_at_once_; }
    void eq_launch(uint32_t out[5]) const { for (int k = 0; k < 5; ++k) out[k] = eq_launch_[k]; }
    void set_tail_hook(std::function<void(hipStream_t)> hook) { tail_hook_ = std::move(hook); }
    void wait_before_next_run(hipEvent_t ev) { head_waits_.push_back(ev); }
    void forget_wait_before_next_run(hipEvent_t ev) { head_waits_.erase(std::remove(head_waits_.begin(), head_waits_.end(), ev), head_waits_.end()); }
    int read_plotter(uint32_t node, uint32_t call, float* left, float* right);
    void ensure_capacity(size_t frames);
    void adopt_state(Graph& old, const int32_t* old_of_new, size_t n);
    struct Perf { bool realtime; int lag; uint32_t tick_rate; uint64_t tick_budget_us, engine_us; };
    Perf performance_info(uint64_t* module_us, size_t cap);
    void set_input_enabled(uint32_t node, uint32_t port, bool enabled);
    void set_video_source(uint32_t node, DFrame* frame, Rational dur, Rational off, bool repeat);
    void set_video_source_band(uint32_t node, uint32_t in_w, uint32_t in_full_h, uint32_t src_row0, uint32_t slice_rows, uint32_t full_w, uint32_t full_h, uint32_t row0, uint32_t band_rows);
    void set_video_source_ring(uint32_t node, DFrame* const* frames, size_t n, Rational dur, Rational off);
    void set_video_source_key(uint32_t node, const mx_video_key_params* params);
    void set_video_source_place(uint32_t node, const mx_video_place_params* params);
    void queue_video_source(uint32_t node, uint64_t tick, DFrame* frame, Rational dur, Rational off);
    void check_video_queue(uint32_t node, uint64_t first_tick) const;
    void check_source_write(uint32_t node, size_t frames) const;
    const Node::MonTick& monitor_tick(uint32_t node, uint32_t tick_in_run);
    void monitor_consume(uint32_t node, uint32_t n_ticks);
    void read_monitor_audio_i16(uint32_t node, int16_t* host, uint32_t n_ticks);
    struct MonitorLayout { uint32_t width, height; size_t frame_bytes, plane_offset[3]; uint32_t stride[3]; };
    MonitorLayout monitor_layout(uint32_t node);
    void read_monitor_video(uint32_t node, uint32_t first_tick, uint32_t n_ticks, uint8_t* frames, uint8_t* present);
    FrameRef video_output(uint32_t node, uint32_t port);
    void rgba_output(uint32_t node, void** dev, int32_t* stride, uint32_t* w, uint32_t* h);

private:
    struct StateLoc { void* p; size_t bytes; };
    std::vector<StateLoc> state_locs(uint32_t node) const;
    void plan_fusion();
    void layout_slab();
    void build_descriptors();
    void upload_group(Group& g);
    void upload_group_one(Group& g, uint32_t parity);
    void run_video_tick(uint64_t t);
    FrameRef keyed_source_frame(uint32_t id, const FrameRef& src);
    FrameRef placed_source_frame(uint32_t id, const FrameRef& src);
    void launch_pending_rgba(Node& n, size_t count, bool with_queued_scales);
    void launch_video_scope(uint32_t tap, const Node::VOut& v);
    void run_span(uint64_t t0, size_t fpc, uint32_t call_off, uint32_t n_calls, uint32_t run_calls);
    void apply_params(uint32_t node, const void* params, size_t len);
    void od_update(Node& n);
    void od_grow(Node& n, uint32_t channels);
    size_t od_offset(const Node& n, uint32_t tick) const;
    struct ProfSpan;
    void launch_outputs(uint64_t t0, uint32_t call_off, uint32_t n_calls, ProfSpan* prof);
    void launch_tap_set(AudioTapSet& s, uint32_t n_calls, ProfSpan* prof);
    void reupload_taps(size_t fpc);
    void refresh_gates(Group& g, uint32_t run_calls);
    uint32_t trigger_of_row(const Group& g, uint32_t row) const;
    void stage_upload(void* dst, const void* src, size_t bytes);
    const float* in_ptr(const Node& n, uint32_t port, bool null_if_disconnected, uint32_t parity) const;
    float* out_ptr(const Node& n, uint32_t port, uint32_t parity) const;

    std::vector<Node> nodes_;
    std::vector<uint32_t> order_;
    std::vector<Group> groups_;
    uint32_t flags_ = 0;
    bool has_video_ = false;
    uint32_t tps_ = 60;
    double sample_rate_ = 44100.0;
    size_t spt_ = 735;
    size_t cap_frames_ = 735;
    int device_ = 0;
    hipStream_t stream_ = nullptr;
    bool own_stream_ = false;
    DevBuf slab_;
    int tail_gi_ = -1;
    bool eq_mode_warned_ = false;
    bool tail_auto_ = false;
    int sin_mode_ = 0;
    uint32_t parity_ = 0;
    hipStream_t tail_stream_ = nullptr;
    hipEvent_t ev_head_done_ = nullptr;
    hipEvent_t ev_tail_done_[2] = {nullptr, nullptr};
    bool tail_pending_[2] = {false, false};
    bool overlap_this_run_ = false;
    struct TailLaunch { const void* desc = nullptr; uint32_t n = 0, max_ch = 0; size_t frames = 0; int dup_mode = 0; hipEvent_t prof_ev = nullptr; };
    struct DeferredTail { bool pending = false; std::vector<TailLaunch> items; uint32_t parity = 0; ProfSpan* prof = nullptr;
                          std::vector<OutRun> outs; std::vector<AudioTapSet*> taps; } deferred_;
    std::function<void(hipStream_t)> tail_hook_;
    std::vector<hipEvent_t> head_waits_;
    uint64_t n_gated_ = 0, n_at_once_ = 0;
    DevBuf gate_flag_; uint32_t gate_seq_ = 0; bool gate_armed_ = false;
    bool gate_test_ = false;
    void flush_deferred_tail(bool gated);
    void end_auto_tail();
    void wait_tail(int parity_or_all);
    const void* desc_of(const Group& g) const { return (parity_ && g.desc_alt.p) ? g.desc_alt.p : g.desc.p; }
    size_t run_off_frames_ = 0;
    uint64_t gates_version_ = 0;
    DevBuf eq_stats_;
    uint32_t eq_launch_[5] = {MX_EQ_LAUNCH_NONE, 0, 0, 0, 0};
    struct Stage { void* host = nullptr; size_t cap = 0; hipEvent_t done = nullptr; bool pending = false; };
    Stage stage_[4]; uint32_t stage_next_ = 0;
    uint32_t prof_runs_count_ = 0;
    std::vector<uint32_t> sched_nodes_;
    std::vector<uint32_t> plotter_nodes_;
    std::vector<uint32_t> video_order_;
    std::vector<uint32_t> od_nodes_;
    size_t tap_fpc_ = 0;
    MeterTaps meters_{*this}; SpectrumTaps spectra_{*this}; LoudnessTaps loudness_{*this}; StereoTaps stereos_{*this}; LimiterTaps limiters_{*this}; TempoTaps tempos_{*this}; TonalityTaps tonalities_{*this};
    const std::array<AudioTapSet*, 7> taps_{&meters_, &spectra_, &loudness_, &stereos_, &limiters_, &tempos_, &tonalities_};
    std::vector<mx_port_ref> scopes_;
    mx_video_scope_params scope_par_{0, 0, 1};
    size_t scope_rec_bytes_ = 0, scope_cap_ = 0;
    DevBuf scope_rec_;
    uint64_t scope_c_ = 0;
    uint32_t scope_n_ = 0;
    uint32_t video_tick_in_run_ = 0;
    bool scope_now_ = false, scope_run_seen_ = false;
    float perf_od_ms_ = 0.f;
    bool prof_this_run_ = false;
    size_t plot_job_off_ = 0;
    size_t zero_off_ = 0;
    size_t slab_floats_ = 0;
    double lo_f_ = 0, hi_f_ = 0;
    DevBuf eq_tabs_;
    DevBuf plot_stage_, plot_jobs_;
    DevBuf conv_stage_;
    size_t last_frames_per_call_ = 0;
    bool prof_on_ = false;
    struct ProfSpan {
        hipEvent_t begin = nullptr;
        std::vector<hipEvent_t> group_end;
        hipEvent_t video_end = nullptr, tail_begin = nullptr;
        hipEvent_t od_end = nullptr, od_tail_end = nullptr;
        hipEvent_t meters_end = nullptr, meters_tail_end = nullptr;
        bool tail_held = false, od = false, od_tail = false, meters = false, meters_tail = false;
        explicit ProfSpan(size_t n_groups);
        ProfSpan(const ProfSpan&) = delete; ProfSpan& operator=(const ProfSpan&) = delete;
        ~ProfSpan();
    };
    std::vector<std::unique_ptr<ProfSpan>> prof_runs_, prof_pool_;
    uint32_t last_calls_ = 0;
    std::vector<float> perf_group_ms_;
    float perf_total_ms_ = 0.f; uint32_t perf_calls_ = 0;
    double perf_last_lag_s_ = -1.0;
};

}
```

mixlab_amd/csrc/mx_k_eq_exact.hip:

```cpp
#include <algorithm>
#include <cmath>

#include "mx_k_eq_common.hpp"

namespace mx {

__device__ __forceinline__ int top_bit64(uint64_t m) { return 63 - __clzll((long long)m); }
__device__ __forceinline__ uint64_t readlane_u64(uint64_t v, int l) {
    const uint32_t lo = (uint32_t)__builtin_amdgcn_readlane((int)(uint32_t)v, l);
    const uint32_t hi = (uint32_t)__builtin_amdgcn_readlane((int)(uint32_t)(v >> 32), l);
    return ((uint64_t)hi << 32) | lo;
}
__device__ __forceinline__ double readlane_f64(double v, int l) {
    return __longlong_as_double((long long)readlane_u64((uint64_t)__double_as_longlong(v), l));
}

template <bool FC>
__global__ __launch_bounds__(256) void k_env_ticks(const EnvTickDesc* __restrict__ descs, uint32_t n_inst, GateBits gates, uint32_t n_calls,
                                                    size_t fpc, uint64_t t0, double sr, double rsr, EnvTick* __restrict__ ticks) {
    const int lane = threadIdx.x & 63;
    const uint32_t inst = blockIdx.x * 4 + (threadIdx.x >> 6);
    if (inst >= n_inst) return;
    const EnvTickDesc d = descs[inst];
    if (!d.state) return;
    uint32_t tag = (uint32_t)__builtin_amdgcn_readfirstlane((int)d.state->tag);
    uint64_t seq = readlane_u64(d.state->seq, 0);
    double off_amp = readlane_f64(d.state->off_amplitude, 0);
    const uint64_t lt = (1ull << lane) - 1ull, le = lt | (1ull << lane);
    for (uint32_t c0 = 0; c0 < n_calls; c0 += 64) {
        const uint32_t c = c0 + (uint32_t)lane;
        const bool valid = c < n_calls;
        const bool b_cur = valid && gate_bit(gates, inst, c);
        const uint64_t m1 = __ballot(b_cur);
        const bool carry_on = tag == 1u;
        const bool b_prev = lane ? ((m1 >> (lane - 1)) & 1ull) != 0 : carry_on;
        const uint64_t R = __ballot(valid && !b_prev && b_cur);
        const uint64_t F = __ballot(valid && b_prev && !b_cur);
        auto t_of = [&](int l) { return t0 + (uint64_t)(c0 + (uint32_t)l) * (uint64_t)fpc; };
        uint32_t my_tag = tag; uint64_t my_seq = seq; double my_off = off_amp;
        const uint64_t Rle = R & le, Fle = F & le;
        if (b_cur) {
            my_tag = 1u;
            if (Rle) my_seq = t_of(top_bit64(Rle));
        } else if (Fle) {
            const int fl = top_bit64(Fle);
            const uint64_t off = t_of(fl);
            const uint64_t Rb = R & ((1ull << fl) - 1ull);
            const uint64_t on = Rb ? t_of(top_bit64(Rb)) : seq;
            my_tag = 2u; my_seq = off;
            my_off = amp_on_ms<FC>(d.p, seq_ms(on, off, sr, rsr));
        }
        if (valid) {
            const uint64_t t = t_of(lane);
            EnvTick k;
            k.seq = my_seq; k.off_amp = my_off; k.tag = my_tag;
            k.flat = env_saturated(d.p, my_tag, my_seq, t, sr, rsr) ? 1u : 0u;
            const float cc = (float)env_amplitude<FC>(d.p, my_tag, my_seq, my_off, t, sr, rsr);
            k.depth = amp_depth<FC>(d.amp_one_minus, d.amp_mod_depth, (double)cc);
            ticks[(size_t)inst * n_calls + c] = k;
        }
        const int last = n_calls - c0 >= 64u ? 63 : (int)(n_calls - c0) - 1;
        tag = (uint32_t)__builtin_amdgcn_readlane((int)my_tag, last);
        seq = readlane_u64(my_seq, last);
        off_amp = readlane_f64(my_off, last);
    }
    if (lane == 0) { d.state->tag = tag; d.state->seq = seq; d.state->off_amplitude = off_amp; }
}
void launch_env_ticks(const EnvTickDesc* d, uint32_t n, const GateBits& gates, uint32_t n_calls, size_t fpc, uint64_t t0, double sample_rate, EnvTick* ticks, hipStream_t s, bool fc) {
    if (!n || !n_calls) return;
    if (fc) hipLaunchKernelGGL(k_env_ticks<true>, dim3((n + 3) / 4), dim3(256), 0, s, d, n, gates, n_calls, fpc, t0, sample_rate, 1.0 / sample_rate, ticks);
    else hipLaunchKernelGGL(k_env_ticks<false>, dim3((n + 3) / 4), dim3(256), 0, s, d, n, gates, n_calls, fpc, t0, sample_rate, 1.0 / sample_rate, ticks);
}

struct EqChunkRec {
    double start[8];
    double end[8];
    uint32_t xmin, xmax;
    uint32_t pad[2];
};

typedef float __attribute__((ext_vector_type(4))) f4v;
typedef float __attribute__((ext_vector_type(2))) f2v;
__device__ __forceinline__ f4v ld_stream4(const float* p) { return __builtin_nontemporal_load(reinterpret_cast<const f4v*>(p)); }

enum { EQM_PLAIN = 0, EQM_AMP_CONST = 1, EQM_AMP_CTL = 2, EQM_AMP_ENV = 3 };

constexpr int EQ_BLK = 16;

struct EnvLane { double A, B, k, m0, depth; uint32_t dt0; uint32_t on; uint32_t flat; uint32_t general;
                 uint32_t k0 = 0; uint64_t t_chunk = 0;  };
__device__ __forceinline__ bool env_params_nice(const EnvParams& p) {
    auto fin = [](double v) { return v == v && fabs(v) < 1.0e300; };
    return fin(p.attack_ms) && fin(p.inv_attack) && fin(p.inv_decay) && fin(p.sustain) && fin(p.one_minus_sustain) && fin(p.inv_release) &&
           p.inv_decay >= 0.0 && p.inv_release >= 0.0;
}
__device__ __forceinline__ EnvLane env_lane_coeffs(const EnvParams& p, const EnvTick& c, uint64_t t_begin, size_t n, bool nice) {
    EnvLane e;
    e.depth = c.depth; e.flat = c.flat; e.on = c.tag == 1u ? 1u : 0u;
    const bool off = c.tag == 2u;
    e.A = e.on ? p.sustain : 0.0; e.B = e.on ? p.one_minus_sustain : (off ? c.off_amp : 0.0);
    e.k = e.on ? p.inv_decay : (off ? p.inv_release : 0.0); e.m0 = e.on ? p.attack_ms : 0.0;
    const uint64_t d0 = t_begin - c.seq;
    e.dt0 = c.tag != 0u ? (uint32_t)d0 : 0u;
    const bool off_ok = !(c.off_amp < 0.0) && (c.off_amp == c.off_amp) && !signbit(c.off_amp) && fabs(c.off_amp) < 1.0e300;
    e.general = (!nice || (c.tag != 0u && ((((d0 + n) >> 32) != 0) || (off && !off_ok)))) ? 1u : 0u;
    return e;
}
template <bool FC>
__device__ __forceinline__ double env_lane_depth(const EnvParams& p, const EnvLane& e, uint32_t k, double one_minus, double mod_depth, double sr, double rsr) {
    const double ms = ms_of_u32(e.dt0 + k, sr, rsr);
    const double tt = e.k * (ms - e.m0);
    const double c = __builtin_fmin(tt, 1.0);
    const double val = mul_add<FC>(e.B, 1.0 - c, e.A);
    const double att = p.inv_attack * ms;
    const double a = (e.on && ms < p.attack_ms) ? att : val;
    const float cc = (float)a;
    return amp_depth<FC>(one_minus, mod_depth, (double)cc);
}

template <int MODE, bool STEREO, int ENVK, bool FC>
__device__ __forceinline__ void eq_spec_span(const EqDesc& d, const EqRun& r, const float* __restrict__ in, float* __restrict__ outm,
                                             const float* __restrict__ ctl, const size_t n, const EnvTick& cur, const EnvLane& el, uint64_t t,
                                             EqPoles& s, uint32_t& xmin, uint32_t& xmax) {
    const double g_lo = d.gain_lo, g_mid = d.gain_mid, g_hi = d.gain_hi, lo_f = r.lo_f, hi_f = r.hi_f;
    const double one_minus = d.amp_one_minus, mod_depth = d.amp_mod_depth, amplitude = d.amp_amplitude;
    const double depth_const = one_minus + mod_depth * 1.0;
    const double rsr = r.rsr;
    uint32_t kk = 0;
    auto fold = [&](float y, float c) -> float {
        if (MODE == EQM_PLAIN) return y;
        double depth;
        if (MODE == EQM_AMP_CONST) depth = depth_const;
        else if (MODE == EQM_AMP_CTL) depth = amp_depth<FC>(one_minus, mod_depth, (double)c);
        else if (ENVK == 1) depth = el.depth;
        else if (ENVK == 2) { depth = env_lane_depth<FC>(d.env, el, kk, one_minus, mod_depth, r.sr, rsr); ++kk; }
        else { depth = env_depth<FC>(d.env, cur, one_minus, mod_depth, t, r.sr, rsr); ++t; }
        return amp_apply(y, depth, amplitude);
    };
    auto track = [&](float x) { const uint32_t b = __float_as_uint(x); xmin = b < xmin ? b : xmin; xmax = b > xmax ? b : xmax; };
    auto put4 = [&](size_t i, const float (&v)[4]) {
        if (STEREO) {
            f4v a = {v[0], v[0], v[1], v[1]}, b = {v[2], v[2], v[3], v[3]};
            __builtin_nontemporal_store(a, reinterpret_cast<f4v*>(outm + 2 * i));
            __builtin_nontemporal_store(b, reinterpret_cast<f4v*>(outm + 2 * i + 4));
        } else {
            f4v a = {v[0], v[1], v[2], v[3]};
            __builtin_nontemporal_store(a, reinterpret_cast<f4v*>(outm + i));
        }
    };
    const size_t n_blk = n / EQ_BLK;
    f4v xa[EQ_BLK / 4], ca[EQ_BLK / 4];
    if (n_blk) {
#pragma unroll
        for (int q = 0; q < EQ_BLK / 4; ++q) { xa[q] = ld_stream4(in + 4 * q); if (MODE == EQM_AMP_CTL) ca[q] = ld_stream4(ctl + 4 * q); }
    }
    for (size_t b = 0; b < n_blk; ++b) {
        f4v xb[EQ_BLK / 4], cb[EQ_BLK / 4];
        const size_t nb = (b + 1 < n_blk ? b + 1 : b) * EQ_BLK;
#pragma unroll
        for (int q = 0; q < EQ_BLK / 4; ++q) { xb[q] = ld_stream4(in + nb + 4 * q); if (MODE == EQM_AMP_CTL) cb[q] = ld_stream4(ctl + nb + 4 * q); }
#pragma unroll
        for (int q = 0; q < EQ_BLK / 4; ++q) {
            float v[4];
#pragma unroll
            for (int e = 0; e < 4; ++e) {
                const float x = xa[q][e];
                track(x);
                v[e] = fold(eq_step<FC>(s, lo_f, hi_f, g_lo, g_mid, g_hi, x), MODE == EQM_AMP_CTL ? ca[q][e] : 0.f);
            }
            put4(b * EQ_BLK + 4 * q, v);
            __builtin_amdgcn_sched_barrier(0);
        }
#pragma unroll
        for (int q = 0; q < EQ_BLK / 4; ++q) { xa[q] = xb[q]; if (MODE == EQM_AMP_CTL) ca[q] = cb[q]; }
    }
    size_t i = n_blk * EQ_BLK;
#pragma unroll 1
    for (; i + 4 <= n; i += 4) {
        const f4v x4 = ld_stream4(in + i);
        f4v c4 = {0.f, 0.f, 0.f, 0.f};
        if (MODE == EQM_AMP_CTL) c4 = ld_stream4(ctl + i);
        float v[4];
#pragma unroll
        for (int e = 0; e < 4; ++e) { track(x4[e]); v[e] = fold(eq_step<FC>(s, lo_f, hi_f, g_lo, g_mid, g_hi, x4[e]), c4[e]); }
        put4(i, v);
    }
#pragma unroll 1
    for (; i < n; ++i) {
        const float x = in[i];
        track(x);
        const float v = fold(eq_step<FC>(s, lo_f, hi_f, g_lo, g_mid, g_hi, x), MODE == EQM_AMP_CTL ? ctl[i] : 0.f);
        if (STEREO) reinterpret_cast<float2*>(outm)[i] = make_float2(v, v); else outm[i] = v;
    }
}

template <int MODE, bool STEREO, bool FC>
__device__ __forceinline__ void eq_spec_chunk(const EqDesc& d, const EqRun& r, const EnvTick* __restrict__ ticks, const size_t begin, const size_t len,
                                              EqPoles& s, uint32_t& xmin, uint32_t& xmax) {
    const float* __restrict__ in = d.in + begin;
// ... 238 lines not shown

template <int SB, bool ALIGN_ROWS = false>
__device__ __forceinline__ void eq_tile_bases(EqTileCtx& c) {
    typedef EqTileGeo<SB> G;
    const int s = c.lane % G::S;
#pragma unroll
    for (int k = 0; k < G::N_INSTR; ++k) {
        const int cj = G::ROWS * k + c.lane / G::S;
        const int pce = s ^ G::sw(cj);
        const long long b = (long long)(c.chunk0 + (uint32_t)cj) * (long long)c.C + 4 * pce - (ALIGN_ROWS ? eq_row_shift(c.chunk0 + (uint32_t)cj, c.C) : 0);
        c.base[k] = (int)(b > 0x3fffffffLL ? 0x3fffffffLL : b);
    }
}
template <int SB>
__device__ __forceinline__ void eq_tile_issue(const EqTileCtx& c, float* buf, int so, const float* src = nullptr ) {
    typedef EqTileGeo<SB> G;
    const float* from = src ? src : c.in;
#pragma unroll
    for (int k = 0; k < G::N_INSTR; ++k) {
        const int idx = min(max(c.base[k] + so, 0), (int)c.F - 4);
        __builtin_amdgcn_global_load_lds((mx_gfp1)(from + (size_t)(uint32_t)idx), (mx_lfp3)(buf + k * 256), 16, 0, 0);
    }
}

struct EqK { double lo_f, hi_f, g_lo, g_mid, g_hi, one_minus, mod_depth, amplitude, sr, rsr; EnvParams env; };
__device__ __forceinline__ double pin_sgpr(double v) { asm volatile("; pinned %0" : "+s"(v)); return v; }
__device__ __forceinline__ EqK eq_constants(const EqDesc& d, const EqRun& r) {
    EqK k;
    k.lo_f = pin_sgpr(r.lo_f); k.hi_f = pin_sgpr(r.hi_f);
    k.g_lo = pin_sgpr(d.gain_lo); k.g_mid = pin_sgpr(d.gain_mid); k.g_hi = pin_sgpr(d.gain_hi);
    k.one_minus = pin_sgpr(d.amp_one_minus); k.mod_depth = pin_sgpr(d.amp_mod_depth); k.amplitude = pin_sgpr(d.amp_amplitude);
    k.sr = pin_sgpr(r.sr); k.rsr = pin_sgpr(r.rsr);
    k.env.attack_ms = pin_sgpr(d.env.attack_ms); k.env.inv_attack = pin_sgpr(d.env.inv_attack); k.env.inv_decay = pin_sgpr(d.env.inv_decay);
    k.env.sustain = pin_sgpr(d.env.sustain); k.env.one_minus_sustain = pin_sgpr(d.env.one_minus_sustain); k.env.inv_release = pin_sgpr(d.env.inv_release);
    return k;
}

template <int SB, int MODE, int ENVK, bool WARM, bool FC, bool LO_ONLY = false>
__device__ __forceinline__ void eq_tile_compute(const EqK& K, float* buf, const int lane, const int so, const int len,
                                                const EnvTick& cur, const EnvLane& el, EqPoles& s, uint32_t& xmin, uint32_t& xmax, const float* cbuf = nullptr ) {
    const double g_lo = K.g_lo, g_mid = K.g_mid, g_hi = K.g_hi, lo_f = K.lo_f, hi_f = K.hi_f;
    const double one_minus = K.one_minus, mod_depth = K.mod_depth, amplitude = K.amplitude;
    const double depth_const = one_minus + mod_depth * 1.0;
    typedef EqTileGeo<SB> G;
    const int sw = G::sw(lane);
    f4v* row = reinterpret_cast<f4v*>(buf + lane * SB);
    f4v x4 = row[0 ^ sw];
#pragma unroll 1
    for (int pce = 0; pce < G::S; ++pce) {
        const f4v xn = row[((pce + 1) & (G::S - 1)) ^ sw];
        if (WARM ? (so + 4 * pce >= len) : (so + 4 * pce < len)) {
            const double dx[4] = {(double)x4[0], (double)x4[1], (double)x4[2], (double)x4[3]};
            if (WARM) {
#pragma unroll
                for (int e = 0; e < 4; ++e) { pump<FC>(lo_f, s.lo, dx[e]); if (!LO_ONLY) pump<FC>(hi_f, s.hi, dx[e]); }
            } else {
                const double hh[4] = {s.h0, s.h1, s.h2, dx[0]};
                f4v v, c4 = {0.f, 0.f, 0.f, 0.f};
                if (MODE == EQM_AMP_CTL) c4 = reinterpret_cast<const f4v*>(cbuf + lane * SB)[pce ^ sw];
#pragma unroll
                for (int e = 0; e < 4; ++e) {
                    const uint32_t b = __float_as_uint(x4[e]); xmin = b < xmin ? b : xmin; xmax = b > xmax ? b : xmax;
                    const float y = eq_step_h<FC>(s, lo_f, hi_f, g_lo, g_mid, g_hi, dx[e], hh[e]);
                    if (MODE == EQM_PLAIN) v[e] = y;
                    else {
                        double depth;
                        const uint32_t kk = (uint32_t)(so + 4 * pce + e);
                        if (MODE == EQM_AMP_CONST) depth = depth_const;
                        else if (MODE == EQM_AMP_CTL) depth = amp_depth<FC>(one_minus, mod_depth, (double)c4[e]);
                        else if (ENVK == 1) depth = el.depth;
                        else if (ENVK == 2) depth = env_lane_depth<FC>(K.env, el, kk - el.k0, one_minus, mod_depth, K.sr, K.rsr);
                        else depth = env_depth<FC>(K.env, cur, one_minus, mod_depth, el.t_chunk + kk, K.sr, K.rsr);
                        v[e] = amp_apply(y, depth, amplitude);
                    }
                }
                row[pce ^ sw] = v;
            }
            s.h0 = dx[1]; s.h1 = dx[2]; s.h2 = dx[3];
        }
        x4 = xn;
    }
}

template <int SB, int MODE, bool FC, bool OUT = true>
__device__ __forceinline__ void eq_tile_compute_range(const EqK& K, float* buf, const int lane, const int so, const int len, const int i_lo, const int i_hi,
                                                      const EnvTick& cur, const uint64_t t_chunk, EqPoles& s, uint32_t& xmin, uint32_t& xmax) {
    typedef EqTileGeo<SB> G;
    const int sw = G::sw(lane);
    f4v* row = reinterpret_cast<f4v*>(buf + lane * SB);
#pragma unroll 1
    for (int pce = 0; pce < G::S; ++pce) {
        const int base = so + 4 * pce;
        if (base + 4 > i_lo && base < i_hi && base < len) {
            f4v v = row[pce ^ sw];
#pragma unroll
            for (int e = 0; e < 4; ++e) {
                if (base + e >= i_lo && base + e < i_hi) {
                    if (OUT) {
                        const uint32_t b = __float_as_uint(v[e]); xmin = b < xmin ? b : xmin; xmax = b > xmax ? b : xmax;
                        const float y = eq_step<FC>(s, K.lo_f, K.hi_f, K.g_lo, K.g_mid, K.g_hi, v[e]);
                        const double depth = env_depth<FC>(K.env, cur, K.one_minus, K.mod_depth, t_chunk + (uint64_t)(base + e), K.sr, K.rsr);
                        v[e] = MODE == EQM_AMP_ENV ? amp_apply(y, depth, K.amplitude) : y;
                    } else {
                        const double x = (double)v[e];
                        pump<FC>(K.lo_f, s.lo, x); pump<FC>(K.hi_f, s.hi, x);
                        s.h0 = s.h1; s.h1 = s.h2; s.h2 = x;
                    }
                }
            }
            if (OUT) row[pce ^ sw] = v;
        }
    }
}

template <int SB, bool STEREO, bool RAGGED = false>
__device__ __forceinline__ void eq_tile_store(const EqTileCtx& c, const float* buf, int so) {
    typedef EqTileGeo<SB> G;
#pragma unroll
    for (int k = 0; k < G::N_INSTR; ++k) {
        const f4v o = *reinterpret_cast<const f4v*>(buf + k * 256 + c.lane * 4);
        const int cj = G::ROWS * k + c.lane / G::S;
        const uint32_t chunk = c.chunk0 + (uint32_t)cj;
        const int idx = c.base[k] + so;
        bool mine = true;
        if (RAGGED) {
            const int i = so + 4 * ((c.lane % G::S) ^ G::sw(cj)) - eq_row_shift(chunk, c.C);
            mine = i >= 0 && i + 4 <= (int)c.C;
        }
        if (mine && chunk < c.n_chunks && idx + 4 <= (int)c.F) {
            if (STEREO) {
                f4v a = {o[0], o[0], o[1], o[1]}, b = {o[2], o[2], o[3], o[3]};
                __builtin_nontemporal_store(a, reinterpret_cast<f4v*>(c.out + 2 * idx));
                __builtin_nontemporal_store(b, reinterpret_cast<f4v*>(c.out + 2 * idx + 4));
            } else {
                __builtin_nontemporal_store(o, reinterpret_cast<f4v*>(c.out + idx));
            }
        }
    }
}

enum { EQ_WPB = 4 };
template <int SB, int KMODE, int KSTEREO, bool FC, int NBUF = 2, bool RT = false>
__global__ __launch_bounds__(64 * EQ_WPB, 4) void k_eq_three_spec_tiled(const EqDesc* __restrict__ descs, const EqState* __restrict__ states, EqRun r, EqSpecPlan plan,
                                                                         uint32_t waves_per_inst, EqChunkRec* __restrict__ recs, uint32_t n_waves) {
    extern __shared__ __attribute__((aligned(16))) float eq_tiles_all[];
    constexpr int EQ_SB = SB, EQ_TILE = EqTileGeo<SB>::TILE;
    constexpr int EQ_TILES_PER_WAVE = (NBUF == 2 || KMODE == EQM_AMP_CTL) ? 2 : 1;
    const uint32_t t_enter = (uint32_t)__builtin_amdgcn_s_memtime();
    if (r.started && blockIdx.x == gridDim.x - 1 && threadIdx.x == 0) __hip_atomic_store(r.started, r.started_seq, __ATOMIC_RELAXED, __HIP_MEMORY_SCOPE_AGENT);
    const uint32_t wib = __builtin_amdgcn_readfirstlane(threadIdx.x >> 6);
    const uint32_t wave_id = blockIdx.x * EQ_WPB + wib;
    if (wave_id >= n_waves) return;
    float* const eq_tiles = eq_tiles_all + wib * (EQ_TILES_PER_WAVE * EQ_TILE);
    const uint32_t inst = wave_id / waves_per_inst;
    const EqDesc& d = descs[inst];
    const EqK K = eq_constants(d, r);
    EqTileCtx c;
    c.in = d.in; c.out = d.out;
    c.chunk0 = (wave_id % waves_per_inst) * 64u; c.n_chunks = plan.n_chunks; c.C = plan.chunk; c.F = (uint32_t)r.frames;
    c.lane = (int)(threadIdx.x & 63u);
    eq_tile_bases<SB, RT>(c);
    const uint32_t j = c.chunk0 + (uint32_t)c.lane;
    const bool active = j < plan.n_chunks;
    const long long begin = (long long)j * c.C;
    const int len = active ? (int)((long long)c.F - begin < (long long)c.C ? (long long)c.F - begin : (long long)c.C) : 0;
    const int len0 = (int)((long long)c.F - (long long)c.chunk0 * c.C < (long long)c.C ? (long long)c.F - (long long)c.chunk0 * c.C : (long long)c.C);
    const int row_shift = RT ? eq_row_shift(j, c.C) : 0;
    const int n_warm = (int)(plan.warm / EQ_SB), n_main = (len0 + (RT ? EQ_SB - 4 : 0) + EQ_SB - 1) / EQ_SB;
    const int total = n_warm + n_main;

    EqPoles s;
#pragma unroll
    for (int k = 0; k < 4; ++k) { s.lo[k] = 0.0; s.hi[k] = 0.0; }
    s.h0 = s.h1 = s.h2 = 0.0;
    const bool from_start = begin <= (long long)plan.warm;
    const int warm_from = from_start ? -(int)begin : -(int)plan.warm;
    if (from_start) {
        const EqState& st = states[inst];
#pragma unroll
        for (int k = 0; k < 4; ++k) { s.lo[k] = st.lo[k]; s.hi[k] = st.hi[k]; }
        s.h0 = st.history[0]; s.h1 = st.history[1]; s.h2 = st.history[2];
    } else if (active) {
        eq_spec_guess<FC>(states[inst], K.lo_f, K.hi_f, d.in[begin - (long long)plan.warm], s);
    }
    uint32_t xmin = 0xffffffffu, xmax = 0u;
    const EnvTick* ticks = r.ticks ? r.ticks + (size_t)inst * r.n_calls : nullptr;
    EnvTick cur{}; EnvLane el{};
    const bool nice = env_params_nice(d.env);
    EqChunkRec* rec = recs + (size_t)inst * plan.n_chunks + (active ? j : 0);

    if constexpr (NBUF == 2) eq_tile_issue<SB>(c, eq_tiles, -(int)plan.warm);
    auto begin_sb = [&](int g) -> float* {
        const int so = (g - n_warm) * EQ_SB;
        if constexpr (NBUF == 1) {
            asm volatile("s_waitcnt lgkmcnt(0)" ::: "memory");
            eq_tile_issue<SB>(c, eq_tiles, so);
            if constexpr (KMODE == EQM_AMP_CTL) { if (so >= 0) eq_tile_issue<SB>(c, eq_tiles + EQ_TILE, so, d.ctl); }
            asm volatile("s_waitcnt vmcnt(0)" ::: "memory");
            return eq_tiles;
        }
        if (g + 1 < total) eq_tile_issue<SB>(c, eq_tiles + ((g + 1) & 1) * EQ_TILE, so + EQ_SB);
        if (g + 1 < total) { if (SB == 32) asm volatile("s_waitcnt vmcnt(8)" ::: "memory"); else asm volatile("s_waitcnt vmcnt(4)" ::: "memory"); }
        else asm volatile("s_waitcnt vmcnt(0)" ::: "memory");
        return eq_tiles + (g & 1) * EQ_TILE;
    };
    const int hi_from = (active && from_start) ? warm_from : -(int)plan.warm_hi;
    int hi_min = hi_from;
#pragma unroll
    for (int m = 32; m >= 1; m >>= 1) hi_min = min(hi_min, __shfl_xor(hi_min, m, 64));
    const int n_lo = max(0, min(n_warm, n_warm + (hi_min - (EQ_SB - 1)) / EQ_SB));
    int g = 0;
    for (; g < n_lo; ++g) {
        float* buf = begin_sb(g);
        eq_tile_compute<SB, EQM_PLAIN, 0, true, FC, true>(K, buf, c.lane, (g - n_warm) * EQ_SB - row_shift, warm_from, cur, el, s, xmin, xmax);
    }
    for (; g < n_warm; ++g) {
        float* buf = begin_sb(g);
        eq_tile_compute<SB, EQM_PLAIN, 0, true, FC>(K, buf, c.lane, (g - n_warm) * EQ_SB - row_shift, warm_from, cur, el, s, xmin, xmax);
    }
    if (!RT && active) {
#pragma unroll
        for (int k = 0; k < 4; ++k) { rec->start[k] = s.lo[k]; rec->start[4 + k] = s.hi[k]; }
    }
    if constexpr (KMODE == EQM_AMP_ENV && RT) {
        const int fpc = (int)r.fpc;
        int tick_i = 0, so0 = 0;
        auto tick_at = [&](int ti) { const size_t tk = ((size_t)begin + (size_t)ti * (size_t)fpc) / r.fpc; return ticks[tk < r.n_calls ? tk : r.n_calls - 1]; };
        const uint64_t t_chunk = r.t0 + (uint64_t)begin;
        auto load_tick = [&]() {
            so0 = tick_i * fpc;
            const EnvTick ct = tick_at(tick_i);
            el = env_lane_coeffs(K.env, ct, t_chunk + (uint64_t)so0, r.fpc, nice);
            el.k0 = (uint32_t)so0; el.t_chunk = t_chunk;
        };
        load_tick();
        {
            float* buf = begin_sb(g);
            const EnvTick cur0 = tick_at(0);
            eq_tile_compute_range<SB, KMODE, FC, false>(K, buf, c.lane, -row_shift, len > 0 ? len : 4, -EQ_SB, 0, cur0, t_chunk, s, xmin, xmax);
            if (active) {
#pragma unroll
                for (int k = 0; k < 4; ++k) { rec->start[k] = s.lo[k]; rec->start[4 + k] = s.hi[k]; }
            }
            eq_tile_compute_range<SB, KMODE, FC>(K, buf, c.lane, -row_shift, len, 0, 0x3fffffff, cur0, t_chunk, s, xmin, xmax);
            eq_tile_store<SB, KSTEREO != 0, true>(c, buf, 0);
            ++g;
        }
        while (g < total) {
            int so_g = (g - n_warm) * EQ_SB;
            const int t_end = so0 + fpc;
            if (so_g + EQ_SB <= t_end) {
                const int envk = __ballot(active && so0 < len && el.general != 0u) != 0ull ? 3 : (__ballot(active && so0 < len && el.flat == 0u) == 0ull ? 1 : 2);
                const int g_int = n_warm + t_end / EQ_SB;
                const int g_end = g_int < total ? g_int : total;
                if (envk == 1) {
                    for (; g < g_end; ++g) { float* buf = begin_sb(g); const int so = (g - n_warm) * EQ_SB; eq_tile_compute<SB, KMODE, 1, false, FC>(K, buf, c.lane, so - row_shift, len, cur, el, s, xmin, xmax); eq_tile_store<SB, KSTEREO != 0, true>(c, buf, so); }
                } else if (envk == 2) {
                    for (; g < g_end; ++g) { float* buf = begin_sb(g); const int so = (g - n_warm) * EQ_SB; eq_tile_compute<SB, KMODE, 2, false, FC>(K, buf, c.lane, so - row_shift, len, cur, el, s, xmin, xmax); eq_tile_store<SB, KSTEREO != 0, true>(c, buf, so); }
                } else {
                    const EnvTick cur3 = tick_at(tick_i);
                    for (; g < g_end; ++g) { float* buf = begin_sb(g); const int so = (g - n_warm) * EQ_SB; eq_tile_compute<SB, KMODE, 3, false, FC>(K, buf, c.lane, so - row_shift, len, cur3, el, s, xmin, xmax); eq_tile_store<SB, KSTEREO != 0, true>(c, buf, so); }
                }
            } else {
                const EnvTick now = tick_at(tick_i), nxt = tick_at(tick_i + 1);
                for (; g < total && so_g - (EQ_SB - 4) < t_end; ++g, so_g += EQ_SB) {
                    float* buf = begin_sb(g);
                    eq_tile_compute_range<SB, KMODE, FC>(K, buf, c.lane, so_g - row_shift, len, -0x3fffffff, t_end, now, t_chunk, s, xmin, xmax);
                    eq_tile_compute_range<SB, KMODE, FC>(K, buf, c.lane, so_g - row_shift, len, t_end, 0x3fffffff, nxt, t_chunk, s, xmin, xmax);
                    eq_tile_store<SB, KSTEREO != 0, true>(c, buf, so_g);
                }
                ++tick_i; load_tick();
            }
        }
    } else if constexpr (KMODE == EQM_AMP_ENV) {
        const int sb_per_tick = (int)(r.fpc / EQ_SB);
        while (g < total) {
            const int so0 = (g - n_warm) * EQ_SB;
            const size_t tk = ((size_t)begin + (size_t)so0) / r.fpc;
            cur = ticks[tk < r.n_calls ? tk : r.n_calls - 1];
            const uint64_t t = r.t0 + (uint64_t)begin + (uint64_t)so0;
            el = env_lane_coeffs(K.env, cur, t, r.fpc, nice);
            el.k0 = (uint32_t)so0; el.t_chunk = r.t0 + (uint64_t)begin;
            const int envk = __ballot(active && so0 < len && el.general != 0u) != 0ull ? 3 : (__ballot(active && so0 < len && el.flat == 0u) == 0ull ? 1 : 2);
            const int g_end = g + sb_per_tick < total ? g + sb_per_tick : total;
            if (envk == 1) {
                for (; g < g_end; ++g) { float* buf = begin_sb(g); const int so = (g - n_warm) * EQ_SB; eq_tile_compute<SB, KMODE, 1, false, FC>(K, buf, c.lane, so, len, cur, el, s, xmin, xmax); eq_tile_store<SB, KSTEREO != 0>(c, buf, so); }
            } else if (envk == 2) {
                for (; g < g_end; ++g) { float* buf = begin_sb(g); const int so = (g - n_warm) * EQ_SB; eq_tile_compute<SB, KMODE, 2, false, FC>(K, buf, c.lane, so, len, cur, el, s, xmin, xmax); eq_tile_store<SB, KSTEREO != 0>(c, buf, so); }
            } else {
                for (; g < g_end; ++g) { float* buf = begin_sb(g); const int so = (g - n_warm) * EQ_SB; eq_tile_compute<SB, KMODE, 3, false, FC>(K, buf, c.lane, so, len, cur, el, s, xmin, xmax); eq_tile_store<SB, KSTEREO != 0>(c, buf, so); }
            }
        }
    } else {
        for (; g < total; ++g) {
            float* buf = begin_sb(g);
            const int so = (g - n_warm) * EQ_SB;
            eq_tile_compute<SB, KMODE, 0, false, FC>(K, buf, c.lane, so, len, cur, el, s, xmin, xmax, KMODE == EQM_AMP_CTL ? buf + EQ_TILE : nullptr);
            eq_tile_store<SB, KSTEREO != 0>(c, buf, so);
        }
    }
    if (active) {
#pragma unroll
        for (int k = 0; k < 4; ++k) { rec->end[k] = s.lo[k]; rec->end[4 + k] = s.hi[k]; }
        rec->xmin = xmin; rec->xmax = xmax;
        uint32_t hw = 0, xcc = 0;
        asm volatile("s_getreg_b32 %0, hwreg(HW_REG_HW_ID)" : "=s"(hw));
        asm volatile("s_getreg_b32 %0, hwreg(HW_REG_XCC_ID)" : "=s"(xcc));
        rec->pad[0] = c.lane == 0 ? t_enter : (c.lane == 1 ? hw : (c.lane == 2 ? xcc : 0u));
        rec->pad[1] = (uint32_t)__builtin_amdgcn_s_memtime();
    }
}

__device__ __forceinline__ bool same4(const double (&a)[4], const double* b) {
    bool eq = true;
#pragma unroll
    for (int k = 0; k < 4; ++k) eq = eq && (__double_as_longlong(a[k]) == __double_as_longlong(b[k]));
    return eq;
}
__device__ __forceinline__ bool same8(const double (&a)[8], const double* b) {
    bool eq = true;
#pragma unroll
    for (int k = 0; k < 8; ++k) eq = eq && (__double_as_longlong(a[k]) == __double_as_longlong(b[k]));
    return eq;
}
__device__ __forceinline__ bool all_nan4(const double (&a)[4]) { return a[0] != a[0] && a[1] != a[1] && a[2] != a[2] && a[3] != a[3]; }
__device__ __forceinline__ bool eq_all_nan(const double (&E)[8]) {
    bool a = true;
#pragma unroll
    for (int k = 0; k < 8; ++k) a = a && (E[k] != E[k]);
    return a;
}
__device__ __forceinline__ double shfl_f64(double v, int src) {
    const uint64_t u = (uint64_t)__double_as_longlong(v);
    const uint32_t lo = (uint32_t)__shfl((int)(uint32_t)u, src, 64), hi = (uint32_t)__shfl((int)(uint32_t)(u >> 32), src, 64);
    return __longlong_as_double((long long)(((uint64_t)hi << 32) | lo));
}
__device__ __forceinline__ bool grp_all(bool c, int g0) { return ((__ballot(c) >> g0) & 0xFull) == 0xFull; }
__device__ __forceinline__ void lds_handover() {
    asm volatile("" ::: "memory");
    __builtin_amdgcn_wave_barrier();
    asm volatile("" ::: "memory");
}
template <bool FC>
__device__ __forceinline__ float eq_out_of(double l, double hp, double h0, double g_lo, double g_mid, double g_hi) {
    const double h = h0 - hp;
    const double mid = h0 - (h + l);
    return band_mix<FC>(l, mid, h, g_lo, g_mid, g_hi);
}
__device__ __forceinline__ f4v eq_ld4(const float* __restrict__ p, size_t i, size_t n) {
    if (i + 4 <= n) return *reinterpret_cast<const f4v*>(p + i);
    f4v v = {0.f, 0.f, 0.f, 0.f};
    if (i < n) v[0] = p[i];
    if (i + 1 < n) v[1] = p[i + 1];
    if (i + 2 < n) v[2] = p[i + 2];
    return v;
}

template <bool FC>
struct EqBlkEmit {
    EqEpi E; double sr, rsr; uint64_t t0; size_t fpc;
    size_t left = 1; uint32_t call = 0, cur_call = 0xffffffffu; EnvTick cur{}; bool env = false;
    __device__ __forceinline__ void init(const EqDesc& d, const EqRun& r, uint32_t inst) {
        E = eq_epi_of(d, r.ticks ? r.ticks + (size_t)inst * r.n_calls : nullptr);
        sr = r.sr; rsr = r.rsr; t0 = r.t0; fpc = r.fpc ? r.fpc : 1;
        env = (E.flags & MX_EQF_ENV) && E.epi == 2u && E.ticks;
    }
    __device__ __forceinline__ void seek(size_t i) { if (env) { call = (uint32_t)(i / fpc); left = fpc - i % fpc; } }
    __device__ __forceinline__ void skip(size_t n) {
        if (!env) return;
        while (n >= left) { n -= left; ++call; left = fpc; }
        left -= n;
    }
    __device__ __forceinline__ void emit(size_t i, float y) {
        float v = y;
        if (E.epi == 2u) {
            double depth;
            if (env) {
                if (call != cur_call) { cur = E.ticks[call]; cur_call = call; }
                depth = env_depth<FC>(E.env, cur, E.amp_one_minus, E.amp_mod_depth, t0 + i, sr, rsr);
                if (--left == 0) { ++call; left = fpc; }
            } else {
                const double m = E.ctl ? (double)E.ctl[i] : 1.0;
                depth = amp_depth<FC>(E.amp_one_minus, E.amp_mod_depth, m);
// ... 314 lines not shown

bool eq_plan_spec(uint32_t n, size_t frames, size_t fpc, double lo_f, double hi_f, EqSpecPlan& plan, bool whole_ticks, bool two_tiles) {
    plan = EqSpecPlan{1u, 0u, 0u, 0u, 0u};
    if (!n || !frames) return false;
    size_t W = std::max(eq_warm_len(lo_f), eq_warm_len(hi_f));
    size_t W_hi = eq_warm_len(hi_f) == (size_t)-1 ? W : (eq_warm_len(hi_f) + 31) / 32 * 32;
    const int force_w = env_int("MX_EQ_SPEC_WARM", 0);
    if (force_w > 0) { W = ((size_t)force_w + 15) / 16 * 16; W_hi = W; }
    if (env_int("MX_EQ_SPEC_WARM_HI_FULL", 0)) W_hi = W;
    if (W == (size_t)-1) return false;
    const int force_c = env_int("MX_EQ_SPEC_CHUNKS", 0);
    if (force_c == 1) return false;
    if (frames < 2 * W || frames < 64) return false;
    size_t unit = (fpc && fpc % 16 == 0 && fpc <= frames / 2) ? fpc : 32;
    if (!whole_ticks && unit % 32) unit = 32;
    if (whole_ticks && fpc >= 32 && fpc % 16 != 0) {
        size_t u = fpc; while (u % 4) u += fpc;
        if (u <= frames / 2) unit = u;
    }
    auto chunk_of = [&](size_t nc) { return ((frames + nc - 1) / nc + unit - 1) / unit * unit; };
    const size_t c_min = std::max<size_t>(unit, 256);
    const size_t nc_max = frames / c_min;
    if (nc_max < 2) return false;
    size_t best;
    if (force_c > 1) best = std::min<size_t>((size_t)force_c, nc_max);
    else {
        auto cost = [&](size_t nc) {
            const double waves = (double)n * (double)((nc + 63) / 64);
            const double Cn = (double)chunk_of(nc), wscale = (double)W / 1280.0;
            if (two_tiles) {
                const double resident = 2560.0, rounds = std::ceil(waves / resident), occ = waves / (rounds * resident);
                return ((double)nc * (Cn + (double)W)) / occ * (1.0 + 0.15 * (rounds - 1.0));
            }
            static const double m_us[5] = {0.0, 0.20, 0.16, 0.153, 0.1542}, warm_us[5] = {0.0, 120.0, 140.0, 120.0, 95.0};
            const double per_simd = waves / 1024.0;
            if (per_simd <= 4.0) {
                const int w = std::max(1, (int)std::ceil(per_simd - 1e-9));
                return (double)w * (Cn * m_us[w] + warm_us[w] * wscale);
            }
            return per_simd * (Cn * m_us[4] + warm_us[4] * wscale) * 0.94;
        };
        best = std::min<size_t>(64, nc_max);
        double best_cost = cost(best);
        for (size_t nc = 128; nc <= nc_max && nc <= 8192; nc += 64) {
            const double c = cost(nc);
            if (c < best_cost * 0.98) { best_cost = c; best = nc; }
        }
        const double seq = (double)frames * 110.0 * std::ceil((double)((n + 63) / 64) / 1024.0);
        const double per_simd = std::max(1.0, (double)n * (double)((best + 63) / 64) / 1024.0);
        const double spec = (double)(chunk_of(best) + W) * (per_simd <= 1.0 ? 260.0 : 190.0 * per_simd);
        if (best < 2 || spec >= seq) return false;
    }
    if (best < 2) return false;
    size_t C = chunk_of(best);
    if (C < c_min) C = (c_min + unit - 1) / unit * unit;
    plan.chunk = (uint32_t)C; plan.warm = (uint32_t)W; plan.warm_hi = (uint32_t)std::min(W, W_hi);
    plan.n_chunks = (uint32_t)((frames + C - 1) / C);
    return plan.n_chunks >= 2;
}

__global__ __launch_bounds__(64) void k_tail_gate(const uint32_t* flag, uint32_t seq, uint32_t limit_ticks) {
    if (threadIdx.x) return;
    const uint64_t t0 = __builtin_amdgcn_s_memrealtime();
    for (;;) {
        const uint32_t v = __hip_atomic_load(flag, __ATOMIC_RELAXED, __HIP_MEMORY_SCOPE_AGENT);
        if ((int32_t)(v - seq) >= 0) break;
        if ((uint64_t)__builtin_amdgcn_s_memrealtime() - t0 > limit_ticks) break;
        __builtin_amdgcn_s_sleep(8);
    }
}
void launch_tail_gate(const uint32_t* flag, uint32_t seq, uint32_t limit_us, hipStream_t s) {
    hipLaunchKernelGGL(k_tail_gate, dim3(1), dim3(64), 0, s, flag, seq, limit_us * 100u);
}

size_t eq_spec_scratch_bytes(uint32_t n, const EqSpecPlan& plan) { return (size_t)n * plan.n_chunks * sizeof(EqChunkRec); }

int eq_epilogue_mode(uint32_t epi, uint32_t flags, bool has_ctl) {
    const int mode = epi != 2u ? EQM_PLAIN : ((flags & MX_EQF_ENV) ? EQM_AMP_ENV : (has_ctl ? EQM_AMP_CTL : EQM_AMP_CONST));
    const int stereo = !(epi == 0u || (flags & MX_EQF_MONO_DUP));
    return mode * 2 + stereo;
}

bool launch_eq_three_spec(const EqDesc* d, EqState* st, uint32_t n, const EqRun& r_in, const EqSpecPlan& plan_in, int uniform_mode, void* scratch, uint64_t* stats, hipStream_t s,
                          uint32_t* launch) {
    if (!n || !r_in.frames) return false;
    EqRun r = r_in; EqSpecPlan plan = plan_in;
    uint32_t tail = (uint32_t)(r_in.frames & 3u);
    if (tail) {
        r.frames = r_in.frames - tail;
        plan.n_chunks = (uint32_t)((r.frames + plan.chunk - 1) / plan.chunk);
        if (plan.n_chunks < 2) { r = r_in; plan = plan_in; tail = 0; }
    }
    uint32_t wpi = (plan.n_chunks + 63) / 64;
    EqChunkRec* recs = (EqChunkRec*)scratch;
    EqSpecPlan plan_t = plan; plan_t.pad = (uint32_t)env_int("MX_EQ_REPAIR_TEST", 0);
    const int no_tiles = env_int("MX_EQ_SPEC_DIRECT", 0);
    const int um = uniform_mode;
    const int sb_env = env_int("MX_EQ_SPEC_SB", 0);
    const int sb_auto = (size_t)n * wpi <= 1024 ? (r.fc ? 16 : 32) : 321;
    const int sb = sb_env == 0 ? sb_auto : (!r.fc && sb_env == 32) ? 32 : (sb_env == 16 ? 16 : 321);
    const bool rt = !no_tiles && (um == 6 || um == 7) && r.fpc >= 64 && r.fpc % 32 != 0 && plan.chunk % r.fpc == 0 && plan.chunk % 4 == 0 && r.frames % 4 == 0 &&
                    plan.warm % 32 == 0 && r.frames < (1ull << 30) && r.frames >= 4;
    const bool ctl_tiled = env_int("MX_EQ_CTL_DIRECT", 0) == 0;
    const bool tiled = rt || (!no_tiles && um >= 0 && (ctl_tiled || (um != 4 && um != 5)) && r.frames % 4 == 0 && plan.chunk % 32 == 0 && plan.warm % 32 == 0 &&
                       r.frames < (1ull << 30) && r.frames >= 4 && ((um != 6 && um != 7) || (r.fpc % 32 == 0 && plan.chunk % r.fpc == 0)));
    if (!tiled && tail) { r = r_in; plan = plan_in; tail = 0; wpi = (plan.n_chunks + 63) / 64; }
    if (tiled) {
        static const int lds_pad = env_int("MX_EQ_SPEC_LDS", 0);
        const uint32_t nwv = n * wpi, nwg = (nwv + EQ_WPB - 1) / EQ_WPB;
        const size_t lds = std::max<size_t>((sb == 321 ? 1 : 2) * 64 * (size_t)(sb == 321 ? 32 : sb) * sizeof(float), (size_t)lds_pad);
#define MX_GT(M, S) { if (sb == 321 && r.fc) hipLaunchKernelGGL((k_eq_three_spec_tiled<32, M, S, true, 1>), dim3(nwg), dim3(64 * EQ_WPB), EQ_WPB * lds, s, d, (const EqState*)st, r, plan, wpi, recs, nwv); \
                      else if (sb == 321) hipLaunchKernelGGL((k_eq_three_spec_tiled<32, M, S, false, 1>), dim3(nwg), dim3(64 * EQ_WPB), EQ_WPB * lds, s, d, (const EqState*)st, r, plan, wpi, recs, nwv); \
                      else if (r.fc) hipLaunchKernelGGL((k_eq_three_spec_tiled<16, M, S, true>), dim3(nwg), dim3(64 * EQ_WPB), EQ_WPB * lds, s, d, (const EqState*)st, r, plan, wpi, recs, nwv); \
                      else if (sb == 32) hipLaunchKernelGGL((k_eq_three_spec_tiled<32, M, S, false>), dim3(nwg), dim3(64 * EQ_WPB), EQ_WPB * lds, s, d, (const EqState*)st, r, plan, wpi, recs, nwv); \
                      else hipLaunchKernelGGL((k_eq_three_spec_tiled<16, M, S, false>), dim3(nwg), dim3(64 * EQ_WPB), EQ_WPB * lds, s, d, (const EqState*)st, r, plan, wpi, recs, nwv); }
        if (um == 4 || um == 5) {
            const size_t lds2 = (size_t)2 * 64 * 32 * sizeof(float);
#define MX_GCT(S, F) hipLaunchKernelGGL((k_eq_three_spec_tiled<32, EQM_AMP_CTL, S, F, 1>), dim3(nwg), dim3(64 * EQ_WPB), EQ_WPB * lds2, s, d, (const EqState*)st, r, plan, wpi, recs, nwv)
            if (um == 4) { if (r.fc) MX_GCT(0, true); else MX_GCT(0, false); } else { if (r.fc) MX_GCT(1, true); else MX_GCT(1, false); }
#undef MX_GCT
        } else
        if (rt) {
            const size_t lds1 = (size_t)64 * 32 * sizeof(float);
#define MX_GRT(S, F) hipLaunchKernelGGL((k_eq_three_spec_tiled<32, EQM_AMP_ENV, S, F, 1, true>), dim3(nwg), dim3(64 * EQ_WPB), EQ_WPB * lds1, s, d, (const EqState*)st, r, plan, wpi, recs, nwv)
            if (um == 6) { if (r.fc) MX_GRT(0, true); else MX_GRT(0, false); } else { if (r.fc) MX_GRT(1, true); else MX_GRT(1, false); }
#undef MX_GRT
        } else
        switch (um) {
        case 0: MX_GT(EQM_PLAIN, 0); break;     case 1: MX_GT(EQM_PLAIN, 1); break;
        case 2: MX_GT(EQM_AMP_CONST, 0); break; case 3: MX_GT(EQM_AMP_CONST, 1); break;
        case 6: MX_GT(EQM_AMP_ENV, 0); break;   default: MX_GT(EQM_AMP_ENV, 1); break;
        }
#undef MX_GT
    } else {
#define MX_GO(M, S) { if (r.fc) hipLaunchKernelGGL((k_eq_three_spec<M, S, true>), dim3(n * wpi), dim3(64), 0, s, d, (const EqState*)st, r, plan, wpi, recs); \
                      else hipLaunchKernelGGL((k_eq_three_spec<M, S, false>), dim3(n * wpi), dim3(64), 0, s, d, (const EqState*)st, r, plan, wpi, recs); }
        switch (uniform_mode) {
        case 0: MX_GO(EQM_PLAIN, 0); break;     case 1: MX_GO(EQM_PLAIN, 1); break;
        case 2: MX_GO(EQM_AMP_CONST, 0); break; case 3: MX_GO(EQM_AMP_CONST, 1); break;
        case 4: MX_GO(EQM_AMP_CTL, 0); break;   case 5: MX_GO(EQM_AMP_CTL, 1); break;
        case 6: MX_GO(EQM_AMP_ENV, 0); break;   case 7: MX_GO(EQM_AMP_ENV, 1); break;
        default: MX_GO(-1, -1); break;
        }
#undef MX_GO
    }
    if (launch) {
        launch[0] = !tiled ? 2u : (um == 4 || um == 5) ? 5u : rt ? 4u : 3u;
        launch[1] = !tiled ? 0u : (um == 4 || um == 5 || rt) ? 321u : (uint32_t)(sb == 321 ? 321 : r.fc ? 16 : sb);
        launch[2] = plan.n_chunks; launch[3] = plan.chunk; launch[4] = plan.warm;
    }
    plan_t.n_chunks = plan.n_chunks;
    if (r.fc) hipLaunchKernelGGL(k_eq_three_repair<true>, dim3(n), dim3(64), 0, s, d, st, r, plan_t, (const EqChunkRec*)recs, (unsigned long long*)stats, tail);
    else hipLaunchKernelGGL(k_eq_three_repair<false>, dim3(n), dim3(64), 0, s, d, st, r, plan_t, (const EqChunkRec*)recs, (unsigned long long*)stats, tail);
    return tiled;
}

}
```

mixlab_amd/csrc/mx_kernels.hpp:

```cpp
#pragma once
#include <hip/hip_runtime.h>
#include <stddef.h>
#include <stdint.h>

namespace mx {

struct AmpDesc { const float* in; const float* ctl;  float* out; double amplitude; double mod_depth; };

struct EnvParams { double attack_ms, inv_attack, inv_decay, sustain, one_minus_sustain, inv_release; };
struct EnvDesc {
    const float* gate; float* out;
    float gate_const; uint32_t use_const;
    EnvParams p;
};
struct EnvState { uint32_t tag; uint32_t pad; uint64_t seq; double off_amplitude; };

struct GateBits { const uint32_t* bits; uint32_t words; uint32_t call_off; };
__host__ __device__ inline bool gate_bit(const GateBits& g, uint32_t inst, uint32_t call) {
    const uint32_t c = g.call_off + call;
    return (g.bits[(size_t)inst * g.words + (c >> 5)] >> (c & 31)) & 1u;
}

struct EnvTick { uint64_t seq; double off_amp; double depth; uint32_t tag; uint32_t flat; };
struct EnvTickDesc { EnvParams p; double amp_one_minus, amp_mod_depth; EnvState* state; };

enum { MX_EQF_MONO_DUP = 1u, MX_EQF_ENV = 2u };
struct EqDesc {
    const float* in; float* out; double gain_lo, gain_mid, gain_hi;
    const float* ctl; double amp_one_minus, amp_mod_depth, amp_amplitude; uint32_t epi; uint32_t flags;
    EnvParams env;
};
struct EqState { double lo[4]; double hi[4]; double history[3]; double pad; };

struct EqScanTab { double pw[2][65][4]; double p2[2][6][4]; double h[2][32][4]; double cz[2][4]; };

struct EqSplit { uint32_t n_split; uint32_t l2_pre; uint32_t stream_out ; uint32_t pad; size_t span; size_t warm; double* zbuf ; double* bound ; EnvState* env_snap ; };
struct EqSpanPow { double lo[4], hi[4]; };

struct FmDesc { const float* in; float* out; double freq_mid, freq_amp; };

struct MixChan { const float* in; double gain;  uint32_t cue; uint32_t dup;  };
struct MixDesc { const MixChan* chans; uint32_t n_ch; uint32_t pad; float* master; float* cue; };

struct OscDesc { float* mono; float* stereo; double freq; uint32_t waveform; uint32_t pad; };

struct PanDesc { const float* l; const float* r; float* out; };
struct SplitDesc { const float* in; float* l; float* r; };

struct TrigDesc { float* out; float value; uint32_t pad; };

struct PlotJob { const float* in; float* left; float* right; };

struct FirDesc { const float* in; float* out; const double* taps; float2* hist; uint32_t n_taps; uint32_t pad; };
struct ResampleDesc { const float* in; float* out; const double* taps ; float2* hist;
                      uint32_t up, down, taps_per_phase, pad; };

void launch_amplifier(const AmpDesc* d, uint32_t n, size_t frames, hipStream_t s, bool fc = false);
void launch_envelope(const EnvDesc* d, EnvState* st, uint32_t n, size_t frames, size_t fpc, const GateBits& gates, uint64_t t0, double sample_rate, hipStream_t s, bool fc = false,
                     void* scratch = nullptr, size_t scratch_bytes = 0 );
size_t envelope_scratch_bytes(uint32_t n, size_t frames);
void launch_env_ticks(const EnvTickDesc* d, uint32_t n, const GateBits& gates, uint32_t n_calls, size_t fpc, uint64_t t0, double sample_rate, EnvTick* ticks, hipStream_t s, bool fc = false);
struct EqRun { size_t frames; size_t fpc ; uint32_t n_calls; uint32_t fc ; uint64_t t0; double sr, rsr , lo_f, hi_f; const EnvTick* ticks ;
               uint32_t* started = nullptr; uint32_t started_seq = 0;  };
void launch_eq_three_exact(const EqDesc* d, EqState* st, uint32_t n, const EqRun& r, void* scratch, hipStream_t s);
bool eq_use_poles_split(uint32_t n, size_t frames);
size_t eq_poles_scratch_bytes(uint32_t n, size_t frames);
int eq_scan_log2l(size_t frames);
void launch_eq_three_scan(const EqDesc* d, EqState* st, uint32_t n, const EqRun& r,
                          const EqScanTab* tabs , const EqSplit& split, const EqSpanPow& pp, hipStream_t s);
struct EqSpecPlan { uint32_t n_chunks; uint32_t chunk; uint32_t warm; uint32_t pad; uint32_t warm_hi ; };
bool eq_plan_spec(uint32_t n, size_t frames, size_t fpc, double lo_f, double hi_f, EqSpecPlan& plan, bool whole_ticks = false ,
                  bool two_tiles = false );
size_t eq_spec_scratch_bytes(uint32_t n, const EqSpecPlan& plan);
void launch_tail_gate(const uint32_t* flag, uint32_t seq, uint32_t limit_us, hipStream_t s);
int eq_epilogue_mode(uint32_t epi, uint32_t flags, bool has_ctl);
bool launch_eq_three_spec(const EqDesc* d, EqState* st, uint32_t n, const EqRun& r, const EqSpecPlan& plan, int uniform_mode ,
                          void* scratch, uint64_t* stats , hipStream_t s,
                          uint32_t* launch = nullptr );
void eq_plan_split(uint32_t n, size_t frames, double lo_f, double hi_f, EqSplit& sp);
void launch_fm_sine(const FmDesc* d, uint32_t n, size_t frames, uint64_t t0, double sample_rate, hipStream_t s, int sin_mode );
void launch_mixer(const MixDesc* d, uint32_t n, uint32_t max_ch , size_t frames,
                  int dup_mode , hipStream_t s);
void launch_oscillator(const OscDesc* d, uint32_t n, size_t frames, uint64_t t0, double sample_rate, hipStream_t s, int sin_mode);
void launch_panner(const PanDesc* d, uint32_t n, size_t frames, hipStream_t s);
void launch_splitter(const SplitDesc* d, uint32_t n, size_t frames, hipStream_t s);
void launch_trigger(const TrigDesc* d, uint32_t n, size_t frames, size_t fpc, const GateBits* gates , hipStream_t s);
void launch_plotter(const PlotJob* d, uint32_t n, size_t spt, hipStream_t s);
void launch_f32_to_i16(const float* in, int16_t* out, size_t n, int dup, hipStream_t s);
void launch_i16_to_f32(const int16_t* in, float* out, size_t n, hipStream_t s);
struct CopyJob { void* dst; const void* src; size_t bytes; };
void launch_copy_jobs(const CopyJob* device_jobs, uint32_t n, hipStream_t s);
void launch_upload(void* dst_device, const void* src_pinned_host, size_t bytes, hipStream_t s);
struct OutState { int64_t last_clip, last_lag; uint32_t clip_status, lag_status; };
struct OutTick { uint8_t clip, clip_status, lag_status, changed; uint32_t channels; };
struct OutRun {
    const float* in; uint32_t dup;
    uint32_t frames, channels;
    int32_t left, right;
    uint32_t n_ticks;
    float* scratch; float* out;
    uint32_t* partial;
    OutState* state; OutTick* rec;
    uint64_t t0; uint32_t spt, rate, lag;
};
uint32_t out_route_blocks(size_t frames_per_tick, uint32_t channels);
void launch_output_device(const OutRun& r, hipStream_t s);
enum : uint32_t { METER_MONO = 0, METER_STEREO = 1, METER_DUP = 2 };
struct TapDesc { const float* p; uint32_t frames, layout, slot, _pad; };
struct MeterDesc { const float* p; uint32_t frames, layout, slot, hold_ticks; float release; uint32_t _pad; };
struct MeterTick { float peak[2], hold[2]; double sum_sq[2]; uint32_t over[2], frames, channels; };
struct MeterHold { float h; uint32_t a; };
struct MeterRun {
    const MeterDesc* desc; uint32_t n;
    uint32_t n_ticks, stride;
    MeterTick* rec; MeterHold* state;
};
void launch_taps(const MeterRun& r, hipStream_t s);
struct SpecRun {
    const TapDesc* desc; uint32_t n;
    uint32_t n_ticks, stride;
    uint32_t n_fft, n_bands;
    const float* window; const float2* twiddle; const uint16_t* edges;
    const float* hist_in; float* hist_out;
    float* rec;
};
void launch_taps(const SpecRun& r, hipStream_t s);
bool spectrum_tables(uint32_t n_fft, float* window, float* twiddle_re, float* twiddle_im);
static constexpr uint32_t LOUD_HIST_TICKS = 1023, LOUD_HIST_FRAMES = 11, LOUD_MAX_FRAMES = 1u << 22;
struct LoudTick { double ksq[2], momentary_sq, short_sq; float true_peak[2]; uint32_t frames, channels; };
struct LoudCoef { double bq[10], carry[16]; };
struct LoudRun {
    const TapDesc* desc; uint32_t n;
    uint32_t n_ticks, stride;
    uint32_t momentary_ticks, short_ticks;
    const LoudCoef* coef;
    const float* interp;
    double* state;
    double* walk; uint32_t walk_ticks;
    const double* ehist_in; double* ehist_out;
    const float* xhist_in; float* xhist_out;
    LoudTick* rec;
};
void launch_taps(const LoudRun& r, hipStream_t s);
bool loudness_tables(double rate, uint32_t frames, double* biquads, double* carry, float* interp);
static constexpr uint32_t STEREO_HIST_TICKS = 1023;
struct StereoTick { double sum_ll, sum_rr, sum_lr, win_ll, win_rr, win_lr; uint32_t frames, nonfinite; };
struct StereoRun {
    const TapDesc* desc; uint32_t n;
    uint32_t n_ticks, stride;
    uint32_t window_ticks;
    const double* hist_in; double* hist_out;
    StereoTick* rec;
    uint32_t grid, zoom_log2, hop, phase;
    uint32_t n_emit, rec_words;
    uint32_t* gon_rec;
    uint32_t* gon_carry;
};
inline size_t stereo_gonio_record_bytes(uint32_t grid) { return 32 + 4 * (size_t)grid * grid; }
void launch_taps(const StereoRun& r, hipStream_t s);
static constexpr uint32_t LIMIT_MAX_LOOKAHEAD = 512, LIMIT_HIST_FRAMES = 2 * LIMIT_MAX_LOOKAHEAD, LIMIT_TILE = 2048, LIMIT_MAX_FRAMES = 1u << 30;
struct LimitDesc { const float* p; uint32_t frames, layout, slot, channels; uint64_t off; };
// ... 81 lines not shown
```

Before: 441.7 million channel-ticks/s.

## Add row-form inline Envelope path to speculative EqThree tiled kernel

```diff
diff --git a/include/mixlab_gpu.h b/include/mixlab_gpu.h
--- a/include/mixlab_gpu.h
+++ b/include/mixlab_gpu.h
@@ -117,6 +117,7 @@
 #define MX_EQ_LAUNCH_CONTROL_TILE 5u
 #define MX_EQ_LAUNCH_SCAN 6u
 int mx_graph_debug_eq_launch(mx_graph* g, uint32_t out[5]);
+int mx_graph_debug_eq_env_rows(mx_graph* g, uint32_t* rows);
 
 int mx_graph_write_source(mx_graph* g, uint32_t node, const float* host_samples, size_t n_ticks);
 int mx_graph_bind_source_device(mx_graph* g, uint32_t node, const void* device_ptr);
diff --git a/mixlab_amd/abi.py b/mixlab_amd/abi.py
--- a/mixlab_amd/abi.py
+++ b/mixlab_amd/abi.py
@@ -113,6 +113,7 @@
 _proto("mx_graph_debug_eq_records", C.c_int, C.c_void_p, C.POINTER(C.c_void_p), C.POINTER(C.c_size_t))
 _proto("mx_graph_debug_tail_releases", C.c_int, C.c_void_p, C.POINTER(C.c_uint64), C.POINTER(C.c_uint64))
 _proto("mx_graph_debug_eq_launch", C.c_int, C.c_void_p, C.POINTER(C.c_uint32))
+_proto("mx_graph_debug_eq_env_rows", C.c_int, C.c_void_p, C.POINTER(C.c_uint32))
 _proto("mx_graph_eq_repair_stats", C.c_int, C.c_void_p, C.POINTER(C.c_uint64))
 _proto("mx_graph_write_source", C.c_int, C.c_void_p, C.c_uint32, C.c_void_p, C.c_size_t)
 _proto("mx_graph_bind_source_device", C.c_int, C.c_void_p, C.c_uint32, C.c_void_p)
@@ -521,6 +522,11 @@
         check(lib.mx_graph_debug_eq_launch(self._h, v))
         return {"form": EQ_LAUNCH.get(v[0], str(v[0])), "super_block": int(v[1]), "n_chunks": int(v[2]), "chunk": int(v[3]), "warm": int(v[4])}
 
+    def debug_eq_env_rows(self) -> bool:
+        v = C.c_uint32()
+        check(lib.mx_graph_debug_eq_env_rows(self._h, C.byref(v)))
+        return bool(v.value)
+
     def debug_eq_records(self):
         p, n = C.c_void_p(), C.c_size_t()
         check(lib.mx_graph_debug_eq_records(self._h, C.byref(p), C.byref(n)))
diff --git a/mixlab_amd/csrc/mx_abi.cpp b/mixlab_amd/csrc/mx_abi.cpp
--- a/mixlab_amd/csrc/mx_abi.cpp
+++ b/mixlab_amd/csrc/mx_abi.cpp
@@ -132,6 +132,10 @@
 
 int mx_graph_debug_eq_launch(mx_graph* g, uint32_t out[5]) {
     return guard([&] { REQUIRE(g && out, "NULL argument"); g->g->eq_launch(out); });
+}
+
+int mx_graph_debug_eq_env_rows(mx_graph* g, uint32_t* rows) {
+    return guard([&] { REQUIRE(g && rows, "NULL argument"); *rows = g->g->eq_env_rows() ? 1u : 0u; });
 }
 
 int mx_graph_eq_repair_stats(mx_graph* g, uint64_t out[8]) {
diff --git a/mixlab_amd/csrc/mx_engine.cpp b/mixlab_amd/csrc/mx_engine.cpp
--- a/mixlab_amd/csrc/mx_engine.cpp
+++ b/mixlab_amd/csrc/mx_engine.cpp
@@ -300,6 +300,7 @@
     }
     { const char* const sm = getenv("MX_SIN_MODE"); sin_mode_ = sm ? atoi(sm) : 0; }
     { const char* const gt = getenv("MX_TAIL_GATE_TEST"); gate_test_ = gt && atoi(gt); }
+    { const char* const er = getenv("MX_EQ_ENV_ROWS"); eq_env_rows_ = !(er && atoi(er) == 0); }
     bool overlap_auto = false;
     {
         const char* const ae = getenv("MX_OVERLAP_AUTO");
@@ -1165,7 +1166,11 @@
                         if (!gate_flag_.p) { gate_flag_.alloc(64); hip_check(hipMemset(gate_flag_.p, 0, 64), "hipMemset"); }
                         r.started = (uint32_t*)gate_flag_.p; r.started_seq = ++gate_seq_; gate_armed_ = true;
                     }
-                    const bool opens_gate = launch_eq_three_spec((const EqDesc*)desc_of(g), (EqState*)g.state.p, n, r, plan, g.eq_mode, g.spec.p, (uint64_t*)eq_stats_.p, stream_, launch);
+                    if (first_eq) {
+                        if (!eq_rows_flag_.p) { eq_rows_flag_.alloc(64); hip_check(hipMemset(eq_rows_flag_.p, 0, 64), "hipMemset"); }
+                        r.env_rows = (uint32_t*)eq_rows_flag_.p; r.env_rows_seq = ++eq_rows_seq_;
+                    }
+                    const bool opens_gate = launch_eq_three_spec((const EqDesc*)desc_of(g), (EqState*)g.state.p, n, r, plan, g.eq_mode, g.spec.p, (uint64_t*)eq_stats_.p, stream_, launch, eq_env_rows_);
                     if (!opens_gate && !gate_test_) gate_armed_ = false;
                     if (deferred_.pending) flush_deferred_tail(true);
                 } else {
@@ -1193,7 +1198,10 @@
                 launch_eq_three_scan((const EqDesc*)desc_of(g), (EqState*)g.state.p, n, r, (const EqScanTab*)eq_tabs_.p, sp, pp, stream_);
                 launch[0] = MX_EQ_LAUNCH_SCAN; launch[2] = sp.n_split; launch[3] = (uint32_t)sp.span; launch[4] = (uint32_t)sp.warm;
             }
-            if (first_eq) { std::copy(launch, launch + 5, eq_launch_); first_eq = false; }
+            if (first_eq) {
+                std::copy(launch, launch + 5, eq_launch_); first_eq = false;
+                if (!r.env_rows) ++eq_rows_seq_;
+            }
             break;
         }
         case MX_KIND_FM_SINE: launch_fm_sine((const FmDesc*)desc_of(g), n, gf, t0, sample_rate_, stream_, sin_mode_); break;
@@ -1615,6 +1623,14 @@
         if (g.kind == MX_KIND_EQ_THREE && g.spec.p) { if (bytes) *bytes = g.spec.bytes; return g.spec.p; }
     if (bytes) *bytes = 0;
     return nullptr;
+}
+
+bool Graph::eq_env_rows() {
+    if (!eq_rows_flag_.p || !eq_rows_seq_) return false;
+    sync();
+    uint32_t v = 0;
+    hip_check(hipMemcpy(&v, eq_rows_flag_.p, sizeof v, hipMemcpyDeviceToHost), "hipMemcpy(eq env rows)");
+    return v == eq_rows_seq_;
 }
 
 float* Graph::output_ptr(uint32_t node, uint32_t port, size_t* fpf, bool stream_ordered_consumer) {
diff --git a/mixlab_amd/csrc/mx_engine.hpp b/mixlab_amd/csrc/mx_engine.hpp
--- a/mixlab_amd/csrc/mx_engine.hpp
+++ b/mixlab_amd/csrc/mx_engine.hpp
@@ -153,6 +153,7 @@
     bool tail_held() const { return deferred_.pending; }
     void tail_releases(uint64_t* gated, uint64_t* at_once) const { if (gated) *gated = n_gated_; if (at_once) *at_once = n_at_once_; }
     void eq_launch(uint32_t out[5]) const { for (int k = 0; k < 5; ++k) out[k] = eq_launch_[k]; }
+    bool eq_env_rows();
     void set_tail_hook(std::function<void(hipStream_t)> hook) { tail_hook_ = std::move(hook); }
     void wait_before_next_run(hipEvent_t ev) { head_waits_.push_back(ev); }
     void forget_wait_before_next_run(hipEvent_t ev) { head_waits_.erase(std::remove(head_waits_.begin(), head_waits_.end(), ev), head_waits_.end()); }
@@ -246,6 +247,8 @@
     uint64_t gates_version_ = 0;
     DevBuf eq_stats_;
     uint32_t eq_launch_[5] = {MX_EQ_LAUNCH_NONE, 0, 0, 0, 0};
+    bool eq_env_rows_ = true;
+    DevBuf eq_rows_flag_; uint32_t eq_rows_seq_ = 0;
     struct Stage { void* host = nullptr; size_t cap = 0; hipEvent_t done = nullptr; bool pending = false; };
     Stage stage_[4]; uint32_t stage_next_ = 0;
     uint32_t prof_runs_count_ = 0;
diff --git a/mixlab_amd/csrc/mx_k_eq_exact.hip b/mixlab_amd/csrc/mx_k_eq_exact.hip
--- a/mixlab_amd/csrc/mx_k_eq_exact.hip
+++ b/mixlab_amd/csrc/mx_k_eq_exact.hip
@@ -1,6 +1,7 @@
 #include <algorithm>
 #include <cmath>
 
+#include "mx_common.hpp"
 #include "mx_k_eq_common.hpp"
 
 namespace mx {
@@ -106,15 +107,20 @@
     e.general = (!nice || (c.tag != 0u && ((((d0 + n) >> 32) != 0) || (off && !off_ok)))) ? 1u : 0u;
     return e;
 }
+enum { ENVP_ANY = 0, ENVP_OFF = 1, ENVP_ON = 2, ENVP_ON_LATE = 3 };
+template <bool FC, int PH = ENVP_ANY>
+__device__ __forceinline__ float env_lane_cc(const EnvParams& p, double A, double B, double k, double m0, bool on, uint32_t dt, double sr, double rsr) {
+    const double ms = ms_of_u32(dt, sr, rsr);
+    const double tt = k * (PH == ENVP_OFF ? ms : ms - m0);
+    const double c = __builtin_fmin(tt, 1.0);
+    const double val = PH == ENVP_OFF ? B * (1.0 - c) : mul_add<FC>(B, 1.0 - c, A);
+    if (PH == ENVP_OFF || PH == ENVP_ON_LATE) return (float)val;
+    const double att = p.inv_attack * ms;
+    return (float)(((PH == ENVP_ON || on) && ms < p.attack_ms) ? att : val);
+}
 template <bool FC>
 __device__ __forceinline__ double env_lane_depth(const EnvParams& p, const EnvLane& e, uint32_t k, double one_minus, double mod_depth, double sr, double rsr) {
-    const double ms = ms_of_u32(e.dt0 + k, sr, rsr);
-    const double tt = e.k * (ms - e.m0);
-    const double c = __builtin_fmin(tt, 1.0);
-    const double val = mul_add<FC>(e.B, 1.0 - c, e.A);
-    const double att = p.inv_attack * ms;
-    const double a = (e.on && ms < p.attack_ms) ? att : val;
-    const float cc = (float)a;
+    const float cc = env_lane_cc<FC>(p, e.A, e.B, e.k, e.m0, e.on != 0u, e.dt0 + k, sr, rsr);
     return amp_depth<FC>(one_minus, mod_depth, (double)cc);
 }
 
@@ -519,6 +525,55 @@
     }
 }
 
+struct EqEnvRow { double off_amp; uint32_t dtk ; uint32_t where ; };
+enum { EQ_ENV_ROW_ENTRIES = 68 };
+template <typename T> __device__ __forceinline__ T* eq_uniform_ptr(T* p) {
+    const uint64_t v = (uint64_t)p;
+    return (T*)(((uint64_t)(uint32_t)__builtin_amdgcn_readfirstlane((int)(uint32_t)(v >> 32)) << 32) | (uint32_t)__builtin_amdgcn_readfirstlane((int)(uint32_t)v));
+}
+__device__ __forceinline__ int eq_rank64(uint64_t m) { return (int)__builtin_amdgcn_mbcnt_hi((uint32_t)(m >> 32), __builtin_amdgcn_mbcnt_lo((uint32_t)m, 0u)); }
+struct EqEnvRowPlan { int p_late, p_early, p_off; };
+__device__ __forceinline__ EqEnvRowPlan eq_env_rows_plan(const EqK& K, EqEnvRow* tab, const EnvLane& el, const bool mine, const int lane) {
+    const bool on = el.on != 0u;
+    const bool early = on && ms_of_u32(el.dt0, K.sr, K.rsr) < K.env.attack_ms;
+    const uint64_t m_late = __ballot(mine && on && !early), m_early = __ballot(mine && early), m_off = __ballot(mine && !on);
+    const int n_late = __builtin_popcountll(m_late), n_early = __builtin_popcountll(m_early), n_off = __builtin_popcountll(m_off);
+    const EqEnvRowPlan plan{(n_late + 1) >> 1, (n_early + 1) >> 1, (n_off + 1) >> 1};
+    const int first = !on ? 2 * (plan.p_late + plan.p_early) : (early ? 2 * plan.p_late : 0);
+    const int n = !on ? n_off : (early ? n_early : n_late);
+    const int rank = eq_rank64(!on ? m_off : (early ? m_early : m_late));
+    if (mine) {
+        const EqEnvRow e{el.B, el.dt0 - el.k0, (uint32_t)(lane * 128) | ((uint32_t)EqTileGeo<32>::sw(lane) << 4)};
+        tab[first + rank] = e;
+        if (rank == n - 1 && (n & 1)) tab[first + rank + 1] = e;
+    }
+    return plan;
+}
+template <bool FC, int PH>
+__device__ __forceinline__ const EqEnvRow* eq_env_row_passes(const EqK& K, char* cbuf, const EqEnvRow* e, const int n, const uint32_t soi, const uint32_t slot) {
+    auto pass = [&](const EqEnvRow& row) {
+        const float cc = PH == ENVP_OFF ? env_lane_cc<FC, ENVP_OFF>(K.env, 0.0, row.off_amp, K.env.inv_release, 0.0, false, row.dtk + soi, K.sr, K.rsr)
+                                        : env_lane_cc<FC, PH>(K.env, K.env.sustain, K.env.one_minus_sustain, K.env.inv_decay, K.env.attack_ms, true, row.dtk + soi, K.sr, K.rsr);
+        *reinterpret_cast<float*>(cbuf + (row.where ^ slot)) = cc;
+    };
+    int q = 0;
+#pragma clang loop vectorize(disable) interleave(disable) unroll(disable)
+    for (; q + 1 < n; q += 2, e += 4) { const EqEnvRow r0 = e[0], r1 = e[2]; pass(r0); pass(r1); }
+    if (q < n) { const EqEnvRow r0 = e[0]; pass(r0); e += 2; }
+    return e;
+}
+template <int SB, bool FC>
+__device__ __forceinline__ void eq_env_rows(const EqK& K, float* cbuf, const EqEnvRow* tab, const EqEnvRowPlan& plan, const int lane, const int so) {
+    static_assert(SB == 32, "a row is the 32 lanes of half a wave");
+    const int i = lane & 31;
+    const uint32_t soi = (uint32_t)(so + i);
+    const uint32_t slot = (uint32_t)(((i >> 2) << 4) | ((i & 3) << 2));
+    const EqEnvRow* e = tab + (lane >> 5);
+    e = eq_env_row_passes<FC, ENVP_ON_LATE>(K, reinterpret_cast<char*>(cbuf), e, plan.p_late, soi, slot);
+    e = eq_env_row_passes<FC, ENVP_ON>(K, reinterpret_cast<char*>(cbuf), e, plan.p_early, soi, slot);
+    eq_env_row_passes<FC, ENVP_OFF>(K, reinterpret_cast<char*>(cbuf), e, plan.p_off, soi, slot);
+}
+
 template <int SB, int MODE, bool FC, bool OUT = true>
 __device__ __forceinline__ void eq_tile_compute_range(const EqK& K, float* buf, const int lane, const int so, const int len, const int i_lo, const int i_hi,
                                                       const EnvTick& cur, const uint64_t t_chunk, EqPoles& s, uint32_t& xmin, uint32_t& xmax) {
@@ -577,23 +632,28 @@
 }
 
 enum { EQ_WPB = 4 };
-template <int SB, int KMODE, int KSTEREO, bool FC, int NBUF = 2, bool RT = false>
+template <int SB, int KMODE, int KSTEREO, bool FC, int NBUF = 2, bool RT = false, bool ROWS = false >
 __global__ __launch_bounds__(64 * EQ_WPB, 4) void k_eq_three_spec_tiled(const EqDesc* __restrict__ descs, const EqState* __restrict__ states, EqRun r, EqSpecPlan plan,
                                                                          uint32_t waves_per_inst, EqChunkRec* __restrict__ recs, uint32_t n_waves) {
     extern __shared__ __attribute__((aligned(16))) float eq_tiles_all[];
     constexpr int EQ_SB = SB, EQ_TILE = EqTileGeo<SB>::TILE;
-    constexpr int EQ_TILES_PER_WAVE = (NBUF == 2 || KMODE == EQM_AMP_CTL) ? 2 : 1;
+    static_assert(!ROWS || (KMODE == EQM_AMP_ENV && !RT && NBUF == 1 && SB == 32), "the row form: the whole-tick inline Envelope over one whole-line tile");
+    constexpr int EQ_TILES_PER_WAVE = (NBUF == 2 || KMODE == EQM_AMP_CTL || ROWS) ? 2 : 1;
+    constexpr int EQ_WAVE_FLOATS = EQ_TILES_PER_WAVE * EQ_TILE + (ROWS ? EQ_ENV_ROW_ENTRIES * (int)(sizeof(EqEnvRow) / sizeof(float)) : 0);
     const uint32_t t_enter = (uint32_t)__builtin_amdgcn_s_memtime();
     if (r.started && blockIdx.x == gridDim.x - 1 && threadIdx.x == 0) __hip_atomic_store(r.started, r.started_seq, __ATOMIC_RELAXED, __HIP_MEMORY_SCOPE_AGENT);
     const uint32_t wib = __builtin_amdgcn_readfirstlane(threadIdx.x >> 6);
     const uint32_t wave_id = blockIdx.x * EQ_WPB + wib;
     if (wave_id >= n_waves) return;
-    float* const eq_tiles = eq_tiles_all + wib * (EQ_TILES_PER_WAVE * EQ_TILE);
-    const uint32_t inst = wave_id / waves_per_inst;
+    float* const eq_tiles = eq_tiles_all + wib * EQ_WAVE_FLOATS;
+    const uint32_t inst = ROWS ? (uint32_t)__builtin_amdgcn_readfirstlane((int)(wave_id / waves_per_inst)) : wave_id / waves_per_inst;
     const EqDesc& d = descs[inst];
     const EqK K = eq_constants(d, r);
     EqTileCtx c;
     c.in = d.in; c.out = d.out;
+    if constexpr (ROWS) {
+        c.out = eq_uniform_ptr(d.out);
+    }
     c.chunk0 = (wave_id % waves_per_inst) * 64u; c.n_chunks = plan.n_chunks; c.C = plan.chunk; c.F = (uint32_t)r.frames;
     c.lane = (int)(threadIdx.x & 63u);
     eq_tile_bases<SB, RT>(c);
@@ -622,9 +682,12 @@
     }
     uint32_t xmin = 0xffffffffu, xmax = 0u;
     const EnvTick* ticks = r.ticks ? r.ticks + (size_t)inst * r.n_calls : nullptr;
+    if constexpr (ROWS) ticks = eq_uniform_ptr(ticks);
     EnvTick cur{}; EnvLane el{};
     const bool nice = env_params_nice(d.env);
-    EqChunkRec* rec = recs + (size_t)inst * plan.n_chunks + (active ? j : 0);
+    EqChunkRec* rec = ROWS ? nullptr : recs + (size_t)inst * plan.n_chunks + (active ? j : 0);
+    EqChunkRec* const recs_inst = ROWS ? eq_uniform_ptr(recs + (size_t)inst * plan.n_chunks) : nullptr;
+    bool rows_ran = false;
 
     if constexpr (NBUF == 2) eq_tile_issue<SB>(c, eq_tiles, -(int)plan.warm);
     auto begin_sb = [&](int g) -> float* {
@@ -655,6 +718,7 @@
         float* buf = begin_sb(g);
         eq_tile_compute<SB, EQM_PLAIN, 0, true, FC>(K, buf, c.lane, (g - n_warm) * EQ_SB - row_shift, warm_from, cur, el, s, xmin, xmax);
     }
+    if constexpr (ROWS) { uint32_t je = active ? j : 0u; asm volatile("; my record %0" : "+v"(je)); rec = recs_inst + je; }
     if (!RT && active) {
 #pragma unroll
         for (int k = 0; k < 4; ++k) { rec->start[k] = s.lo[k]; rec->start[4 + k] = s.hi[k]; }
@@ -713,15 +777,38 @@
         const int sb_per_tick = (int)(r.fpc / EQ_SB);
         while (g < total) {
             const int so0 = (g - n_warm) * EQ_SB;
-            const size_t tk = ((size_t)begin + (size_t)so0) / r.fpc;
+            uint32_t jt = j;
+            if constexpr (ROWS) asm volatile("; my chunk %0" : "+v"(jt));
+            const long long begin_t = (long long)jt * c.C;
+            const size_t tk = ((size_t)begin_t + (size_t)so0) / r.fpc;
             cur = ticks[tk < r.n_calls ? tk : r.n_calls - 1];
-            const uint64_t t = r.t0 + (uint64_t)begin + (uint64_t)so0;
+            const uint64_t t = r.t0 + (uint64_t)begin_t + (uint64_t)so0;
             el = env_lane_coeffs(K.env, cur, t, r.fpc, nice);
-            el.k0 = (uint32_t)so0; el.t_chunk = r.t0 + (uint64_t)begin;
+            el.k0 = (uint32_t)so0; el.t_chunk = r.t0 + (uint64_t)begin_t;
             const int envk = __ballot(active && so0 < len && el.general != 0u) != 0ull ? 3 : (__ballot(active && so0 < len && el.flat == 0u) == 0ull ? 1 : 2);
             const int g_end = g + sb_per_tick < total ? g + sb_per_tick : total;
             if (envk == 1) {
                 for (; g < g_end; ++g) { float* buf = begin_sb(g); const int so = (g - n_warm) * EQ_SB; eq_tile_compute<SB, KMODE, 1, false, FC>(K, buf, c.lane, so, len, cur, el, s, xmin, xmax); eq_tile_store<SB, KSTEREO != 0>(c, buf, so); }
+            } else if (ROWS && envk == 2) {
+                if constexpr (ROWS) {
+                    float* const cbuf = eq_tiles + EQ_TILE;
+                    EqEnvRow* const tab = reinterpret_cast<EqEnvRow*>(eq_tiles + 2 * EQ_TILE);
+                    const EqEnvRowPlan rows = eq_env_rows_plan(K, tab, el, active && so0 < len && el.flat == 0u, c.lane);
+                    const float cc = env_lane_cc<FC>(K.env, el.A, el.B, el.k, el.m0, el.on != 0u, el.dt0, K.sr, K.rsr);
+                    const f4v cc4 = {cc, cc, cc, cc};
+#pragma unroll
+                    for (int q = 0; q < EQ_SB / 4; ++q) reinterpret_cast<f4v*>(cbuf + c.lane * EQ_SB)[q] = cc4;
+                    rows_ran = true;
+                    for (; g < g_end; ++g) {
+                        const int so = (g - n_warm) * EQ_SB;
+                        asm volatile("s_waitcnt lgkmcnt(0)" ::: "memory");
+                        eq_tile_issue<SB>(c, eq_tiles, so);
+                        eq_env_rows<SB, FC>(K, cbuf, tab, rows, c.lane, so);
+                        asm volatile("s_waitcnt vmcnt(0)" ::: "memory");
+                        eq_tile_compute<SB, EQM_AMP_CTL, 0, false, FC>(K, eq_tiles, c.lane, so, len, cur, el, s, xmin, xmax, cbuf);
+                        eq_tile_store<SB, KSTEREO != 0>(c, eq_tiles, so);
+                    }
+                }
             } else if (envk == 2) {
                 for (; g < g_end; ++g) { float* buf = begin_sb(g); const int so = (g - n_warm) * EQ_SB; eq_tile_compute<SB, KMODE, 2, false, FC>(K, buf, c.lane, so, len, cur, el, s, xmin, xmax); eq_tile_store<SB, KSTEREO != 0>(c, buf, so); }
             } else {
@@ -736,6 +823,12 @@
             eq_tile_store<SB, KSTEREO != 0>(c, buf, so);
         }
     }
+    if constexpr (ROWS) {
+        uint32_t je = active ? j : 0u;
+        asm volatile("; my record %0" : "+v"(je));
+        rec = recs_inst + je;
+    }
+    if (ROWS && rows_ran && r.env_rows && c.lane == 0) __hip_atomic_store(r.env_rows, r.env_rows_seq, __ATOMIC_RELAXED, __HIP_MEMORY_SCOPE_AGENT);
     if (active) {
 #pragma unroll
         for (int k = 0; k < 4; ++k) { rec->end[k] = s.lo[k]; rec->end[4 + k] = s.hi[k]; }
@@ -1216,7 +1309,7 @@
 }
 
 bool launch_eq_three_spec(const EqDesc* d, EqState* st, uint32_t n, const EqRun& r_in, const EqSpecPlan& plan_in, int uniform_mode, void* scratch, uint64_t* stats, hipStream_t s,
-                          uint32_t* launch) {
+                          uint32_t* launch, bool env_rows) {
     if (!n || !r_in.frames) return false;
     EqRun r = r_in; EqSpecPlan plan = plan_in;
     uint32_t tail = (uint32_t)(r_in.frames & 3u);
@@ -1233,6 +1326,7 @@
     const int sb_env = env_int("MX_EQ_SPEC_SB", 0);
     const int sb_auto = (size_t)n * wpi <= 1024 ? (r.fc ? 16 : 32) : 321;
     const int sb = sb_env == 0 ? sb_auto : (!r.fc && sb_env == 32) ? 32 : (sb_env == 16 ? 16 : 321);
+    const bool rows = env_rows && !no_tiles && (um == 6 || um == 7) && sb == 321 && (size_t)n * wpi <= 2048 && r.fpc % 32 == 0;
     const bool rt = !no_tiles && (um == 6 || um == 7) && r.fpc >= 64 && r.fpc % 32 != 0 && plan.chunk % r.fpc == 0 && plan.chunk % 4 == 0 && r.frames % 4 == 0 &&
                     plan.warm % 32 == 0 && r.frames < (1ull << 30) && r.frames >= 4;
     const bool ctl_tiled = env_int("MX_EQ_CTL_DIRECT", 0) == 0;
@@ -1260,6 +1354,14 @@
             if (um == 6) { if (r.fc) MX_GRT(0, true); else MX_GRT(0, false); } else { if (r.fc) MX_GRT(1, true); else MX_GRT(1, false); }
 #undef MX_GRT
         } else
+        if (rows) {
+            const size_t lds_r = (size_t)2 * 64 * 32 * sizeof(float) + EQ_ENV_ROW_ENTRIES * sizeof(EqEnvRow);
+#define MX_GRW(S, F) { auto* const kern = k_eq_three_spec_tiled<32, EQM_AMP_ENV, S, F, 1, false, true>; \
+                       hip_check(hipFuncSetAttribute((const void*)kern, hipFuncAttributeMaxDynamicSharedMemorySize, (int)(EQ_WPB * lds_r)), "hipFuncSetAttribute(EqThree row form: dynamic LDS)"); \
+                       hipLaunchKernelGGL(kern, dim3(nwg), dim3(64 * EQ_WPB), EQ_WPB * lds_r, s, d, (const EqState*)st, r, plan, wpi, recs, nwv); }
+            if (um == 6) { if (r.fc) MX_GRW(0, true) else MX_GRW(0, false) } else { if (r.fc) MX_GRW(1, true) else MX_GRW(1, false) }
+#undef MX_GRW
+        } else
         switch (um) {
         case 0: MX_GT(EQM_PLAIN, 0); break;     case 1: MX_GT(EQM_PLAIN, 1); break;
         case 2: MX_GT(EQM_AMP_CONST, 0); break; case 3: MX_GT(EQM_AMP_CONST, 1); break;
diff --git a/mixlab_amd/csrc/mx_kernels.hpp b/mixlab_amd/csrc/mx_kernels.hpp
--- a/mixlab_amd/csrc/mx_kernels.hpp
+++ b/mixlab_amd/csrc/mx_kernels.hpp
@@ -61,7 +61,8 @@
 size_t envelope_scratch_bytes(uint32_t n, size_t frames);
 void launch_env_ticks(const EnvTickDesc* d, uint32_t n, const GateBits& gates, uint32_t n_calls, size_t fpc, uint64_t t0, double sample_rate, EnvTick* ticks, hipStream_t s, bool fc = false);
 struct EqRun { size_t frames; size_t fpc ; uint32_t n_calls; uint32_t fc ; uint64_t t0; double sr, rsr , lo_f, hi_f; const EnvTick* ticks ;
-               uint32_t* started = nullptr; uint32_t started_seq = 0;  };
+               uint32_t* started = nullptr; uint32_t started_seq = 0;
+               uint32_t* env_rows = nullptr; uint32_t env_rows_seq = 0;  };
 void launch_eq_three_exact(const EqDesc* d, EqState* st, uint32_t n, const EqRun& r, void* scratch, hipStream_t s);
 bool eq_use_poles_split(uint32_t n, size_t frames);
 size_t eq_poles_scratch_bytes(uint32_t n, size_t frames);
@@ -76,7 +77,8 @@
 int eq_epilogue_mode(uint32_t epi, uint32_t flags, bool has_ctl);
 bool launch_eq_three_spec(const EqDesc* d, EqState* st, uint32_t n, const EqRun& r, const EqSpecPlan& plan, int uniform_mode ,
                           void* scratch, uint64_t* stats , hipStream_t s,
-                          uint32_t* launch = nullptr );
+                          uint32_t* launch = nullptr ,
+                          bool env_rows = true );
 void eq_plan_split(uint32_t n, size_t frames, double lo_f, double hi_f, EqSplit& sp);
 void launch_fm_sine(const FmDesc* d, uint32_t n, size_t frames, uint64_t t0, double sample_rate, hipStream_t s, int sin_mode );
 void launch_mixer(const MixDesc* d, uint32_t n, uint32_t max_ch , size_t frames,
```

Measured after the change: 471.8 million channel-ticks/s, median of 6. 6.8% higher.
